# sczhou/CodeFormer

Measured on AMD Instinct MI355X. Metric: aligned 512x512 faces/sec (whole node) at w=0.5, higher is better.
Workload: dtype f32; 1 GPU; BASELINE config 2 (IEEE fp32 arithmetic): 16 faces/GPU, w=0.5, adain, seed-0 random-init weights; global_batch=16, parallelism=single GPU, precision=fp32

## Files before the change

### codeformer_amd/archs/vqgan_arch.py

```python
import torch
import torch.nn.functional as F
from torch import nn

from .. import ops
from ..ops import EPI_RESIDUAL, PRO_AFFINE, PRO_AFFINE_SWISH
from ..utils.logger import get_root_logger
from ..utils.registry import ARCH_REGISTRY
from .hip_module import HipModule

GN_GROUPS = 32
GN_EPS = 1e-6


def normalize(in_channels):
    return nn.GroupNorm(num_groups=GN_GROUPS, num_channels=in_channels, eps=GN_EPS, affine=True)


def swish(x):
    return x * torch.sigmoid(x)


def _gn_tables(norm, *xs, act_growth=None):
    return ops.groupnorm_tables(list(xs), norm.weight, norm.bias, norm.eps, norm.num_groups, act_growth=act_growth)


class VectorQuantizer(HipModule):

    def __init__(self, codebook_size, emb_dim, beta):
        super().__init__()
        self.codebook_size = codebook_size
        self.emb_dim = emb_dim
        self.beta = beta
        self.embedding = nn.Embedding(self.codebook_size, self.emb_dim)
        self.embedding.weight.data.uniform_(-1.0 / self.codebook_size, 1.0 / self.codebook_size)

    def _stats(self, z_q, z, idx, mean_distance):
        enc = torch.zeros(idx.shape[0], self.codebook_size, dtype=z.dtype, device=z.device)
        enc.scatter_(1, idx.view(-1, 1), 1)
        loss = torch.mean((z_q - z) ** 2) * (1.0 + self.beta)
        e_mean = enc.mean(dim=0)
        perplexity = torch.exp(-torch.sum(e_mean * torch.log(e_mean + 1e-10)))
        return loss, {'perplexity': perplexity, 'min_encodings': enc, 'min_encoding_indices': idx.view(-1, 1),
                      'mean_distance': mean_distance}

    def forward(self, z):
        if not z.is_cuda:
            return self.forward_host(z)
        with torch.no_grad():
            B, C, H, W = z.shape
            zt = ops.to_nhwc(z.float()).view(B * H * W, C)
            cb = self.embedding.weight
            pw = self._packed('codebook', lambda: ops.pack_weight(cb), cb)
            idx, _, (scores, zz, ee) = ops.vq_nearest(zt, cb, pw)
            zq_t = ops.codebook_gather(idx, cb, B, H * W)
            z_q = ops.to_nchw(zq_t.view(B, H, W, C))
            loss, stats = self._stats(z_q, z, idx, zz.mean() + ee.mean() - 2.0 * scores.mean())
            return z_q, loss, stats

    def forward_host(self, z):
        zp = z.permute(0, 2, 3, 1).contiguous()
        zf = zp.view(-1, self.emb_dim)
        w = self.embedding.weight
        d = (zf ** 2).sum(dim=1, keepdim=True) + (w ** 2).sum(1) - 2 * torch.matmul(zf, w.t())
        idx = torch.argmin(d, dim=1)
        z_q = w[idx].view(zp.shape)
        z_q = (zp + (z_q - zp).detach()).permute(0, 3, 1, 2).contiguous()
        loss, stats = self._stats(z_q, z, idx, torch.mean(d))
        return z_q, loss, stats

    def get_codebook_feat(self, indices, shape):
        if not indices.is_cuda:
            z_q = self.embedding.weight[indices.view(-1)]
            if shape is not None:
                z_q = z_q.view(shape).permute(0, 3, 1, 2).contiguous()
            return z_q
        with torch.no_grad():
            idx = indices.reshape(-1).contiguous()
            if shape is None:
                return ops.codebook_gather(idx, self.embedding.weight, 1, idx.numel()).view(idx.numel(), -1)
            B, H, W, C = shape
            return ops.to_nchw(ops.codebook_gather(idx, self.embedding.weight, B, H * W).view(B, H, W, C))


class Downsample(HipModule):

    def __init__(self, in_channels):
        super().__init__()
        self.conv = nn.Conv2d(in_channels, in_channels, kernel_size=3, stride=2, padding=0)

    def forward_nhwc(self, x, bf16=False):
        cin, cout = self.conv.in_channels, self.conv.out_channels
        if int(bf16) in (2,) + ops.SPLIT_CODES and ops.split_s2_ok(cin, cout, x.shape[1], x.shape[2]):
            pw = self._packed(('conv', 's2'), lambda: ops.pack_weight(self.conv.weight, self.conv.bias, bf16=ops.SPLIT, stride2=True),
                              self.conv.weight, self.conv.bias)
            return ops.conv2d(x, pw, stride=2, emit_stats=True, act=ops.act_scale(x) if ops.needs_act_scale(pw) else None)
        return ops.conv2d(x, self._pw_conv('conv'), stride=2, emit_stats=True)

    def forward_host(self, x):
        return self.conv(F.pad(x, (0, 1, 0, 1), mode='constant', value=0))


class Upsample(HipModule):

    def __init__(self, in_channels):
        super().__init__()
        self.conv = nn.Conv2d(in_channels, in_channels, kernel_size=3, stride=1, padding=1)

    def forward_nhwc(self, x, bf16=False):
        if int(bf16) == 2:
            bf16 = ops.SPLIT
        c = self.conv.in_channels
        if int(bf16) == ops.WINOGRAD_F43 and x.dtype == torch.float32 and ops.f43_up_ok(c, self.conv.out_channels, 2 * x.shape[1], 2 * x.shape[2]):
            pw = self._packed(('conv', 'f43up'), lambda: ops.pack_weight(self.conv.weight, self.conv.bias, bf16=ops.WF43F), self.conv.weight, self.conv.bias)
            return ops.conv2d(x, pw, upsample=True, emit_stats=True)
        pw = self._pw_conv('conv', bf16, up2x=True, hw=x.shape[1:3])
        return ops.conv2d(x, pw, upsample=True, emit_stats=True, act=ops.act_scale(x) if ops.needs_act_scale(pw) else None)

    def forward_host(self, x):
        return self.conv(F.interpolate(x, scale_factor=2.0, mode='nearest'))


class ResBlock(HipModule):

    def __init__(self, in_channels, out_channels=None):
        super().__init__()
        self.in_channels = in_channels
        self.out_channels = in_channels if out_channels is None else out_channels
        self.norm1 = normalize(in_channels)
        oc = self.out_channels
        self.conv1 = nn.Conv2d(in_channels, oc, kernel_size=3, stride=1, padding=1)
        self.norm2 = normalize(oc)
        self.conv2 = nn.Conv2d(oc, oc, kernel_size=3, stride=1, padding=1)
        if self.in_channels != oc:
            self.conv_out = nn.Conv2d(in_channels, oc, kernel_size=1, stride=1, padding=0)

    def forward_nhwc(self, x, x2=None, bf16=False):
        xs = (x,) if x2 is None else (x, x2)
        sc, sh = _gn_tables(self.norm1, *xs, act_growth=4.0 if self._skip_streams(x, x2, bf16) else None)
        hw = x.shape[1:3]
        npix = hw[0] * hw[1]
        code1 = self._range_code(self.norm1, bf16, npix * self.in_channels // GN_GROUPS)
        code2 = self._range_code(self.norm2, bf16, npix * self.out_channels // GN_GROUPS)
        h = ops.conv2d(x, self._pw_conv('conv1', code1, hw=hw, c_split=None if x2 is None else x.shape[3]), x2=x2, prologue=PRO_AFFINE_SWISH, scale=sc, shift=sh, emit_stats=True)
        sc, sh = _gn_tables(self.norm2, h)
        if self.in_channels != self.out_channels:
            skip = self._skip_nhwc(x, x2, bf16)
        else:
            skip = x
        return ops.conv2d(h, self._pw_conv('conv2', code2, hw=hw), prologue=PRO_AFFINE_SWISH, scale=sc, shift=sh,
                          epilogue=EPI_RESIDUAL, res=skip, emit_stats=True)

    def _skip_streams(self, x, x2, code):
        if self.in_channels == self.out_channels:
            return False
        c_split = None if x2 is None else x.shape[3]
        stored = x.dtype == torch.bfloat16 and getattr(x, '_cf_stats', None) is not None and (x2 is None or getattr(x2, '_cf_stats', None) is not None)
        return bool((int(code) in (2,) + ops.SPLIT_CODES or stored) and ops.RANGE_SCALE and
                    ops.split_1x1_ok(self.in_channels, self.out_channels, x.shape[1], x.shape[2], c_split))

    def _skip_nhwc(self, x, x2, code):
        if self._skip_streams(x, x2, code):
            pw = self._packed(('conv_out', 'f16x2'), lambda: ops.pack_weight(self.conv_out.weight, self.conv_out.bias, bf16=ops.SPLIT),
                              self.conv_out.weight, self.conv_out.bias)
            return ops.conv2d(x, pw, x2=x2, act=ops.act_scale(x, x2))
        return ops.conv2d(x, self._pw_conv('conv_out'), x2=x2)

    def forward_host(self, x_in):
        x = self.conv1(swish(self.norm1(x_in)))
        x = self.conv2(swish(self.norm2(x)))
        if self.in_channels != self.out_channels:
            x_in = self.conv_out(x_in)
        return x + x_in


class AttnBlock(HipModule):

    def __init__(self, in_channels):
        super().__init__()
        self.in_channels = in_channels
        self.norm = normalize(in_channels)
        self.q = nn.Conv2d(in_channels, in_channels, kernel_size=1, stride=1, padding=0)
        self.k = nn.Conv2d(in_channels, in_channels, kernel_size=1, stride=1, padding=0)
        self.v = nn.Conv2d(in_channels, in_channels, kernel_size=1, stride=1, padding=0)
        self.proj_out = nn.Conv2d(in_channels, in_channels, kernel_size=1, stride=1, padding=0)

    def forward_nhwc(self, x):
        B, H, W, C = x.shape
        if H * W != 256:
            raise ValueError(f'AttnBlock HIP path is built for 16x16 feature maps (got {H}x{W})')
        sc, sh = _gn_tables(self.norm, x)
        qkv_w = (self.q.weight, self.k.weight, self.v.weight)
        qkv_b = (self.q.bias, self.k.bias, self.v.bias)
        pw = self._packed('qkv', lambda: ops.pack_weight_cat(qkv_w, qkv_b), *qkv_w, *qkv_b)
        qkv = ops.conv2d(x, pw, prologue=PRO_AFFINE, scale=sc, shift=sh).view(B * 256, 3 * C)
        o = ops.attention(qkv[:, :C], qkv[:, C:2 * C], qkv[:, 2 * C:], B, 1, C, int(C) ** (-0.5))
        return ops.conv2d(o.view(B, H, W, C), self._pw_conv('proj_out'), epilogue=EPI_RESIDUAL, res=x, emit_stats=True)

    def forward_host(self, x):
        h_ = self.norm(x)
        q, k, v = self.q(h_), self.k(h_), self.v(h_)
        b, c, h, w = q.shape
        w_ = torch.bmm(q.reshape(b, c, h * w).permute(0, 2, 1), k.reshape(b, c, h * w)) * (int(c) ** (-0.5))
        w_ = F.softmax(w_, dim=2).permute(0, 2, 1)
        h_ = torch.bmm(v.reshape(b, c, h * w), w_).reshape(b, c, h, w)
        return x + self.proj_out(h_)


class _Conv3x3(HipModule):

    def __init__(self, cin, cout):
        super().__init__()
        conv = nn.Conv2d(cin, cout, kernel_size=3, stride=1, padding=1)
        self.weight, self.bias = conv.weight, conv.bias
        self.in_channels, self.out_channels = cin, cout

    def pw(self, bf16=False):
        return self._packed(('w', int(bf16)), lambda: ops.pack_weight(self.weight, self.bias, bf16=int(bf16)), self.weight,
                            self.bias)

    def forward_nhwc(self, x, bf16=False, **kw):
        plain = not kw.get('out_nchw') and not kw.get('in_nchw')
        if kw.get('img_in') is not None:
            h, w = kw['img_in'].shape[1], kw['img_in'].shape[2]
        else:
            h, w = (x.shape[2], x.shape[3]) if kw.get('in_nchw') else (x.shape[1], x.shape[2])
        unnormalised = plain and kw.get('prologue', ops.PRO_NONE) in (ops.PRO_NONE, ops.PRO_LEAKY)
        if unnormalised and int(bf16) == 2:
            bf16 = ops.SPLIT
        code = ops.conv_code(bf16, self.in_channels, self.out_channels, h, w, plain=plain)
        pw = self.pw(code)
        if unnormalised and ops.needs_act_scale(pw):
            kw['act'] = ops.act_scale(x)
        return ops.conv2d(x, pw, **kw)

    def forward_host(self, x):
        return F.conv2d(x, self.weight, self.bias, stride=1, padding=1)


class _GroupNorm(nn.GroupNorm):

    def forward(self, x):
        if x.is_cuda:
            xn = ops.to_nhwc(x.float())
            sc, sh = ops.groupnorm_tables([xn], self.weight, self.bias, self.eps, self.num_groups)
            B, C = sc.shape
            return x * sc.view(B, C, 1, 1) + sh.view(B, C, 1, 1)
        return super().forward(x)


def _run_blocks_nhwc(blocks, x, taps=None, first_nchw=False, last_nchw=False, bf16=False, storage_bf16=False, img_in=False, img_out=None):
    pending = None
    n = len(blocks)
    for i, blk in enumerate(blocks):
        if storage_bf16 and int(bf16) == 1 and isinstance(blk, Upsample) and x.dtype == torch.float32 and \
                4 * x.shape[1] * x.shape[2] > ops.TOKEN_IMAGE_MAX:
            x = ops.to_bf16(x)
        if isinstance(blk, _GroupNorm):
            pending = ops.groupnorm_tables([x], blk.weight, blk.bias, blk.eps, blk.num_groups) + (blk,)
        elif isinstance(blk, _Conv3x3):
            kw = {}
            code = bf16
            if pending is not None:
                kw.update(prologue=PRO_AFFINE, scale=pending[0], shift=pending[1])
                code = blk._range_code(pending[2], bf16, x.shape[1] * x.shape[2] * x.shape[3] // pending[2].num_groups)
                pending = None
            if i == 0 and first_nchw:
                kw['in_nchw'] = True
                if img_in:
                    x, kw['img_in'] = None, x
            if i == n - 1 and last_nchw:
                kw['out_nchw'] = True
                if img_out is not None:
                    kw['img_out'] = img_out
            kw['emit_stats'] = i != n - 1
            x = blk.forward_nhwc(x, bf16=code, **kw)
        else:
            if pending is not None:
                raise RuntimeError('GroupNorm must be followed by a conv in the block list')
            x = blk.forward_nhwc(x, bf16=bf16) if isinstance(blk, (ResBlock, Upsample, Downsample)) else blk.forward_nhwc(x)
        if taps and i in taps:
            r = taps[i](x)
            if r is not None:
                x = r
    return x


class Encoder(HipModule):

    def __init__(self, in_channels, nf, emb_dim, ch_mult, num_res_blocks, resolution, attn_resolutions):
        super().__init__()
        self.nf = nf
        self.num_resolutions = len(ch_mult)
        self.num_res_blocks = num_res_blocks
        self.resolution = resolution
        self.attn_resolutions = attn_resolutions
        res = resolution
        widths = [nf * m for m in (1,) + tuple(ch_mult)]
        seq = [_Conv3x3(in_channels, nf)]
        ch = nf
        for level in range(self.num_resolutions):
            ch = widths[level]
            for _ in range(num_res_blocks):
                seq.append(ResBlock(ch, widths[level + 1]))
                ch = widths[level + 1]
                if res in attn_resolutions:
                    seq.append(AttnBlock(ch))
            if level != self.num_resolutions - 1:
                seq.append(Downsample(ch))
                res //= 2
        seq += [ResBlock(ch, ch), AttnBlock(ch), ResBlock(ch, ch), _GroupNorm(GN_GROUPS, ch, eps=GN_EPS, affine=True),
                _Conv3x3(ch, emb_dim)]
        self.blocks = nn.ModuleList(seq)

    def forward(self, x):
        if not x.is_cuda:
            return self.forward_host(x)
        with torch.no_grad():
            return ops.to_nchw(self.forward_nhwc(x.float().contiguous()))

    def forward_nhwc(self, x_nchw, taps=None, bf16=False, img_u8=False):
        return _run_blocks_nhwc(self.blocks, x_nchw, taps, first_nchw=True, bf16=bf16, img_in=img_u8)

    def forward_host(self, x):
        for blk in self.blocks:
            x = blk(x)
        return x


class Generator(HipModule):

    def __init__(self, nf, emb_dim, ch_mult, res_blocks, img_size, attn_resolutions):
        super().__init__()
        self.nf = nf
        self.ch_mult = ch_mult
        self.num_resolutions = len(self.ch_mult)
        self.num_res_blocks = res_blocks
        self.resolution = img_size
        self.attn_resolutions = attn_resolutions
        self.in_channels = emb_dim
        self.out_channels = 3
        ch = nf * ch_mult[-1]
        res = img_size // 2 ** (self.num_resolutions - 1)
        seq = [_Conv3x3(emb_dim, ch), ResBlock(ch, ch), AttnBlock(ch), ResBlock(ch, ch)]
        for level in reversed(range(self.num_resolutions)):
            width = nf * ch_mult[level]
            for _ in range(res_blocks):
                seq.append(ResBlock(ch, width))
                ch = width
                if res in attn_resolutions:
                    seq.append(AttnBlock(ch))
            if level != 0:
                seq.append(Upsample(ch))
                res *= 2
        seq += [_GroupNorm(GN_GROUPS, ch, eps=GN_EPS, affine=True), _Conv3x3(ch, self.out_channels)]
        self.blocks = nn.ModuleList(seq)

    def forward(self, x):
        if not x.is_cuda:
            return self.forward_host(x)
        with torch.no_grad():
            return self.forward_nhwc(ops.to_nhwc(x.float()))

    def forward_nhwc(self, x, taps=None, bf16=False, storage_bf16=False, img_out=None):
        return _run_blocks_nhwc(self.blocks, x, taps, last_nchw=True, bf16=bf16, storage_bf16=storage_bf16, img_out=img_out)

    def forward_host(self, x):
        for blk in self.blocks:
            x = blk(x)
        return x


@ARCH_REGISTRY.register()
class VQAutoEncoder(HipModule):

    def __init__(self, img_size, nf, ch_mult, quantizer='nearest', res_blocks=2, attn_resolutions=[16],
                 codebook_size=1024, emb_dim=256, beta=0.25, gumbel_straight_through=False, gumbel_kl_weight=1e-8,
                 model_path=None):
        super().__init__()
        logger = get_root_logger()
        self.in_channels = 3
        self.nf = nf
        self.n_blocks = res_blocks
        self.codebook_size = codebook_size
        self.embed_dim = emb_dim
        self.ch_mult = ch_mult
        self.resolution = img_size
        self.attn_resolutions = attn_resolutions
        self.quantizer_type = quantizer
        self.encoder = Encoder(self.in_channels, nf, emb_dim, ch_mult, res_blocks, img_size, attn_resolutions)
        if quantizer == 'nearest':
            self.beta = beta
            self.quantize = VectorQuantizer(codebook_size, emb_dim, beta)
        else:
            raise NotImplementedError(f"quantizer '{quantizer}' is not part of the MI355X inference path")
        self.generator = Generator(nf, emb_dim, ch_mult, res_blocks, img_size, attn_resolutions)
        if model_path is not None:
            chkpt = torch.load(model_path, map_location='cpu')
            key = 'params_ema' if 'params_ema' in chkpt else ('params' if 'params' in chkpt else None)
            if key is None:
                raise ValueError('Wrong params!')
            self.load_state_dict(chkpt[key])
            logger.info(f'vqgan is loaded from: {model_path} [{key}]')

    def forward(self, x):
        x = self.encoder(x)
        quant, codebook_loss, quant_stats = self.quantize(x)
        x = self.generator(quant)
        return x, codebook_loss, quant_stats
```

### codeformer_amd/csrc/cf_wf43.hip

```cpp
#include <cstdlib>
#include <cstring>
#include <type_traits>

#include "cf_conv_parts.h"




namespace {

constexpr int F4_TH = 16, F4_TW = 16;
constexpr int F4_PW = F4_TW + 2;
constexpr int F4_NPIX = (F4_TH + 2) * F4_PW;
constexpr int F4_SLOTS = F4_NPIX + 4;
constexpr int F4_DUMMY = F4_NPIX;
constexpr int F4_NT = 16;
constexpr int F4_PATCH_FLOATS = F4_SLOTS * CF_BK;
constexpr int F4_PS = F4_NT * CF_BK;
constexpr int F4_V_FLOATS = 36 * F4_PS;
constexpr int F4_M_FLOATS = 36 * 8 * 64;
constexpr int F4_TAB = 256;
constexpr int F4_TAB_32 = 512;
constexpr int F4_LDS_FLOATS = 2 * F4_PATCH_FLOATS + F4_V_FLOATS + 2 * F4_TAB;
static_assert(F4_M_FLOATS <= 2 * F4_PATCH_FLOATS + F4_V_FLOATS, "epilogue staging must fit the patch buffers + V");
static_assert(F4_LDS_FLOATS * 4 <= 81920, "LDS budget of two workgroups per CU");
constexpr int F4_LDS_FLOATS_16 = 2 * F4_M_FLOATS;
static_assert(F4_LDS_FLOATS_16 >= F4_LDS_FLOATS && F4_LDS_FLOATS_16 * 4 <= 163840, "LDS budget of the 16-wave form");
constexpr int F4_LDS_FLOATS_32 = 2 * F4_SLOTS * 32 + 36 * F4_NT * 32 + 2 * F4_TAB_32;
static_assert(F4_LDS_FLOATS_32 >= F4_LDS_FLOATS_16 && F4_LDS_FLOATS_32 * 4 <= 163840, "LDS budget of the 32-channel-slab form");

typedef _Float16 f4_f16x4 __attribute__((ext_vector_type(4)));
typedef float f4_f32x2 __attribute__((ext_vector_type(2)));
typedef unsigned f4_u32x4 __attribute__((ext_vector_type(4)));
typedef unsigned f4_u32x2 __attribute__((ext_vector_type(2)));

__device__ __forceinline__ __amdgpu_buffer_rsrc_t f4_rsrc(const void* p, unsigned bytes) {
  return __builtin_amdgcn_make_buffer_rsrc(const_cast<void*>(p), 0, bytes, 0x00020000);
}
__device__ __forceinline__ f32x4 f4_ld128(__amdgpu_buffer_rsrc_t r, unsigned voff, unsigned soff) {
  return __builtin_bit_cast(f32x4, __builtin_amdgcn_raw_buffer_load_b128(r, (int)voff, (int)soff, 0));
}
__device__ __forceinline__ f4_f32x2 f4_ld64(__amdgpu_buffer_rsrc_t r, unsigned voff, unsigned soff) {
  return __builtin_bit_cast(f4_f32x2, __builtin_amdgcn_raw_buffer_load_b64(r, (int)voff, (int)soff, 0));
}
__device__ __forceinline__ void f4_st64(f4_f32x2 v, __amdgpu_buffer_rsrc_t r, unsigned voff, unsigned soff) {
  __builtin_amdgcn_raw_buffer_store_b64(__builtin_bit_cast(f4_u32x2, v), r, (int)voff, (int)soff, 0);
}

struct F4Args {
  const float* in0;
  const float* in1;
  int c0, c1, cin, nchunks;
  int batch, h, w;
  int cout;
  int prologue, epilogue;
  const float* pro_scale;
  const float* pro_shift;
  const float* weight;
  const float* bias;
  const float* res;
  const float* sft_scale;
  float sft_w;
  float acc_scale;
  const float* act_scale;
  float* out;
  double* stats_out;
  int stats_cpg, nparts;
  int tiles_x, tiles_per_img, ntn;
  int nt_out;
};
static_assert(sizeof(F4Args) == 160, "the kernarg block keeps its size: it feeds the register allocation of every instantiation");

__device__ __forceinline__ int f4_vs(int ty) { return (0x78 >> (2 * ty)) & 3; }

__device__ __forceinline__ unsigned f4_vu(unsigned lq, unsigned p, unsigned t) { return (lq & 1u) + 2u * (((t >> 1) + 4u * (lq >> 1) + p) & 7u); }

template <int PRO, int EPI, int NW, int KS, bool F32, bool UP = false>
__global__ __launch_bounds__(NW * 64, 4) void wf43_kernel(const F4Args a) {
  static_assert(!UP || (F32 && PRO == CF_PRO_NONE && EPI == CF_EPI_NONE), "the upsampling gather: fp32 operands, no prologue, no epilogue operand");
  static_assert(KS == 16 || (KS == 32 && NW == 16), "32-channel slabs need the LDS of the 16-wave form");
  constexpr int F4_THREADS = NW * 64;
  constexpr int F4_BN = NW * 8;
  constexpr int TWV = KS / 4;
  constexpr int QPP = KS / 4;
  constexpr int GT = F4_THREADS - TWV * 64;
  constexpr int F4_APT = 384 * QPP / GT;
  constexpr int PSTEP = GT / QPP;
  constexpr int SLOTB = KS * 4;
  constexpr int PATCHF = F4_SLOTS * KS;
  constexpr int PSK = F4_NT * KS;
  extern __shared__ __attribute__((aligned(16))) float smem[];
  float* const V = smem + 2 * PATCHF;
  constexpr int VBUF = 36 * PSK;
  constexpr int TABN = KS == 32 ? F4_TAB_32 : F4_TAB;
  float* const tab = V + VBUF;

  const int tid = threadIdx.x;
  const int lane = tid & 63;
  const int wave = __builtin_amdgcn_readfirstlane(tid >> 6);

  const int bid = cf_xcd_tile(blockIdx.x, gridDim.x);
  const int ntile = bid % a.ntn;
  const int mt = bid / a.ntn;
  const int n0 = ntile * F4_BN;
  const int b = mt / a.tiles_per_img;
  const int rt = mt - b * a.tiles_per_img;
  const int tyw = rt / a.tiles_x;
  const int y0 = tyw * F4_TH;
  const int x0 = (rt - tyw * a.tiles_x) * F4_TW;
  const int n = a.cin / KS;

  constexpr bool affine = PRO == CF_PRO_AFFINE || PRO == CF_PRO_AFFINE_SWISH;
  if (affine) {
    for (int i = tid; i < a.cin; i += F4_THREADS) {
      tab[i] = a.pro_scale[(size_t)b * a.cin + i];
      tab[TABN + i] = a.pro_shift[(size_t)b * a.cin + i];
    }
  }
  float act_s, act_is, act_s02;
  cf_act_scales<!affine>(a.act_scale, b, act_s, act_is, act_s02);

  const int pix_origin = (y0 - 1) * a.w + (x0 - 1);
  auto item = [&](unsigned u, int j, unsigned& rel, bool& valid) __attribute__((always_inline)) {
    const unsigned p = u + (unsigned)(PSTEP * j);
    const unsigned hy = (p * 3641u) >> 16;
    const unsigned hx = p - 18u * hy;
    const int iy = y0 - 1 + (int)hy, ix = x0 - 1 + (int)hx;
    valid = (int)(p < (unsigned)F4_NPIX) & (int)((unsigned)iy < (unsigned)a.h) & (int)((unsigned)ix < (unsigned)a.w);
    if constexpr (UP) {
      const unsigned sy = valid ? (unsigned)iy : (unsigned)(y0 + 8), sx = valid ? (unsigned)ix : (unsigned)(x0 + 8);
      rel = (sy >> 1) * ((unsigned)a.w >> 1) + (sx >> 1);
    } else {
      rel = valid ? hy * (unsigned)a.w + hx : (unsigned)(9 * a.w + 9);
    }
  };
  const size_t img0 = (size_t)b * a.h * a.w;
  const unsigned img_px = (unsigned)(a.h * a.w);
  const size_t img0_in = UP ? img0 / 4 : img0;
  const unsigned img_px_in = UP ? img_px / 4 : img_px;
  const __amdgpu_buffer_rsrc_t rs_in0 = f4_rsrc(a.in0 + img0_in * a.c0, img_px_in * (unsigned)a.c0 * 4u);
  const __amdgpu_buffer_rsrc_t rs_in1 = f4_rsrc(a.c1 ? a.in1 + img0_in * a.c1 : a.in0, img_px_in * (unsigned)a.c1 * 4u);
  constexpr bool HALVES = F4_APT >= 6;
  constexpr int RAN = HALVES ? F4_APT / 2 : F4_APT;
  f32x4 ra[RAN], rb[HALVES ? RAN : 1];
  auto load_A_range = [&](int chunk, auto j0c, auto j1c) __attribute__((always_inline)) {
    constexpr int J0 = decltype(j0c)::value, J1 = decltype(j1c)::value;
    const int c = chunk * KS;
    const bool first = c < a.c0;
    const unsigned cs = (unsigned)(first ? a.c0 : a.c1);
    const unsigned soff = (unsigned)(first ? c : c - a.c0) * 4u;
    unsigned tl = (unsigned)tid - (unsigned)(TWV * 64);
    asm volatile("" : "+v"(tl));
    const unsigned k4x = (tl % (unsigned)QPP) * 4u;
#pragma unroll
    for (int j = J0; j < J1; ++j) {
      unsigned rel;
      bool valid;
      item(tl / (unsigned)QPP, j, rel, valid);
      const unsigned voff = (__umul24(UP ? rel : (unsigned)(pix_origin + (int)rel), cs) + k4x) * 4u;
      (HALVES && j >= RAN ? rb[j % RAN] : ra[j % RAN]) = first ? f4_ld128(rs_in0, voff, soff) : f4_ld128(rs_in1, voff, soff);
    }
  };
  auto load_A = [&](int chunk) __attribute__((always_inline)) { load_A_range(chunk, std::integral_constant<int, 0>{}, std::integral_constant<int, F4_APT>{}); };
  auto store_patch_range = [&](int chunk, auto j0c, auto j1c) __attribute__((always_inline)) {
    constexpr int J0 = decltype(j0c)::value, J1 = decltype(j1c)::value;
    unsigned tl = (unsigned)tid - (unsigned)(TWV * 64);
    asm volatile("" : "+v"(tl));
    const unsigned k4 = tl % (unsigned)QPP, slot = tl / (unsigned)QPP;
    char* const pb = reinterpret_cast<char*>(smem + (chunk & 1) * PATCHF) + (((slot & ~3u) | ((slot ^ (slot >> 2)) & 3u)) * (unsigned)SLOTB + k4 * 16u);
    f32x4 sc = {1.f, 1.f, 1.f, 1.f}, sh = {0.f, 0.f, 0.f, 0.f};
    if (affine) {
      sc = *reinterpret_cast<const f32x4*>(tab + chunk * KS + k4 * 4);
      sh = *reinterpret_cast<const f32x4*>(tab + TABN + chunk * KS + k4 * 4);
    }
#pragma unroll
    for (int j = J0; j < J1; ++j) {
      unsigned rel;
      bool valid;
      item(slot, j, rel, valid);
      const f32x4 v = cf_pro_apply4<PRO, true>(HALVES && j >= RAN ? rb[j % RAN] : ra[j % RAN], sc, sh, act_s, act_s02, valid);
      if (j < F4_APT - 1 || slot + (unsigned)(PSTEP * j) < (unsigned)F4_NPIX) *reinterpret_cast<f32x4*>(pb + j * (PSTEP * SLOTB)) = v;
    }
  };

  auto store_patch = [&](int chunk) __attribute__((always_inline)) { store_patch_range(chunk, std::integral_constant<int, 0>{}, std::integral_constant<int, F4_APT>{}); };

  const int tg = (wave >> (KS == 32 ? 2 : 1)) & 1;
  float* t_hi;
  float* t_lo;
  auto row_pass = [&](const f4_f32x2 (&zz)[6], int pos) __attribute__((always_inline)) {
    f4_f32x2 v[6];
    v[0] = (zz[0] + zz[4]) * 0.25f - zz[2] * 1.0625f;
    const f4_f32x2 e1 = zz[4] * 0.25f - zz[2];
    const f4_f32x2 o1 = zz[3] * 0.125f - zz[1] * 0.5f;
    v[1] = e1 + o1;
    v[2] = e1 - o1;
    const f4_f32x2 e2 = zz[4] * 0.5f - zz[2] * 0.125f;
    const f4_f32x2 o2 = zz[3] - zz[1] * 0.25f;
    v[3] = e2 + o2;
    v[4] = e2 - o2;
    v[5] = (zz[1] + zz[5]) * 0.25f - zz[3] * 1.0625f;
#pragma unroll
    for (int nu = 0; nu < 6; ++nu) {
      if (F32) {
        t_hi[(pos + nu) * PSK] = v[nu][0];
        t_lo[(pos + nu) * PSK] = v[nu][1];
      } else {
        float hi, lo;
        cf_split_pair(v[nu][0], v[nu][1], hi, lo);
        t_hi[(pos + nu) * PSK] = hi;
        t_lo[(pos + nu) * PSK] = lo;
      }
    }
  };
  auto transform = [&](int chunk, auto mid) __attribute__((always_inline)) {
    const char* const pb = reinterpret_cast<const char*>(smem + (chunk & 1) * PATCHF);
    unsigned ln = (unsigned)lane;
    asm volatile("" : "+v"(ln));
    const unsigned t_tile = KS == 32 ? 4u * (unsigned)(wave & 3) + (ln >> 4) : 8u * (unsigned)(wave & 1) + (ln >> 3);
    const unsigned t_cp = KS == 32 ? ln & 15u : ln & 7u;
    const unsigned t_ty = t_tile >> 2, t_tx = t_tile & 3u;
    constexpr unsigned SH = KS == 32 ? 7 : 6;
    const unsigned t_base = (4u << SH) * (18u * t_ty + t_tx) + t_cp * 8u;
    const unsigned tb0 = 2u * t_ty + t_tx;
    unsigned tk[4];
#pragma unroll
    for (int k = 0; k < 4; ++k) tk[k] = t_base | (((tb0 + k) & 3u) << SH);
    if (F32) {
      const unsigned lq0 = (2u * t_cp) & 3u, j = t_cp >> 1;
      if (KS == 32) {
        t_hi = V + (tg * 18) * PSK + t_tile * 32 + f4_vu(lq0, j >> 1, t_tile) * 2u + (j & 1u);
        t_lo = V + (tg * 18) * PSK + t_tile * 32 + f4_vu(lq0 + 1u, j >> 1, t_tile) * 2u + (j & 1u);
      } else {
        t_hi = V + (tg * 18) * PSK + t_tile * CF_BK + ((lq0 ^ (unsigned)f4_vs((int)t_ty)) << 2) + j;
        t_lo = V + (tg * 18) * PSK + t_tile * CF_BK + (((lq0 + 1u) ^ (unsigned)f4_vs((int)t_ty)) << 2) + j;
      }
    } else if (KS == 32) {
      const unsigned lq = t_cp >> 2, e = t_cp & 3u;
      t_hi = V + (tg * 18) * PSK + t_tile * 32 + f4_vu(lq, e >> 1, t_tile) * 2u + (e & 1u);
      t_lo = V + (tg * 18) * PSK + t_tile * 32 + f4_vu(lq, 2u + (e >> 1), t_tile) * 2u + (e & 1u);
    } else {
      t_hi = V + (tg * 18) * PSK + t_tile * CF_BK + (((t_cp >> 1) ^ (unsigned)f4_vs((int)t_ty)) << 2) + (t_cp & 1u);
      t_lo = t_hi + 2;
    }
    auto px = [&](int r, int j) __attribute__((always_inline)) {
      const int q = 2 * r + j;
      return *reinterpret_cast<const f4_f32x2*>(pb + (4 << SH) * (4 * r + (q >> 2)) + (tk[q >> 2] ^ (((unsigned)q & 3u) << SH)));
    };
    if (tg == 0) {
      {
        f4_f32x2 z[6];
#pragma unroll
        for (int j = 0; j < 6; ++j) z[j] = (px(0, j) + px(4, j)) * 0.25f - px(2, j) * 1.0625f;
        __builtin_amdgcn_sched_barrier(0);
        row_pass(z, 0);
      }
      __builtin_amdgcn_sched_barrier(0);
      {
        f4_f32x2 zp[6], zm[6];
#pragma unroll
        for (int j = 0; j < 6; ++j) {
          const f4_f32x2 e = px(4, j) * 0.25f - px(2, j);
          const f4_f32x2 o = px(3, j) * 0.125f - px(1, j) * 0.5f;
          zp[j] = e + o;
          zm[j] = e - o;
          if (j == 2) __builtin_amdgcn_sched_barrier(0);
        }
        __builtin_amdgcn_sched_barrier(0);
        row_pass(zp, 6);
        __builtin_amdgcn_sched_barrier(0);
        mid();
        __builtin_amdgcn_sched_barrier(0);
        row_pass(zm, 12);
      }
    } else {
      {
        f4_f32x2 z[6];
#pragma unroll
        for (int j = 0; j < 6; ++j) z[j] = (px(1, j) + px(5, j)) * 0.25f - px(3, j) * 1.0625f;
        __builtin_amdgcn_sched_barrier(0);
        row_pass(z, 12);
      }
      __builtin_amdgcn_sched_barrier(0);
      {
        f4_f32x2 zp[6], zm[6];
#pragma unroll
        for (int j = 0; j < 6; ++j) {
          const f4_f32x2 e = px(4, j) * 0.5f - px(2, j) * 0.125f;
          const f4_f32x2 o = px(3, j) - px(1, j) * 0.25f;
          zp[j] = e + o;
          zm[j] = e - o;
          if (j == 2) __builtin_amdgcn_sched_barrier(0);
        }
        __builtin_amdgcn_sched_barrier(0);
        row_pass(zp, 0);
        __builtin_amdgcn_sched_barrier(0);
        mid();
        __builtin_amdgcn_sched_barrier(0);
        row_pass(zm, 6);
      }
    }
  };

  const int m_g = wave / (NW / 2), m_nb = wave % (NW / 2);
  f32x4 acc[18];
#pragma unroll
  for (int i = 0; i < 18; ++i) acc[i] = f32x4{0.f, 0.f, 0.f, 0.f};
  const __amdgpu_buffer_rsrc_t rs_w = f4_rsrc(a.weight, 36u * (unsigned)a.cin * (unsigned)a.cout * 4u);
  const unsigned w_pos = (unsigned)a.cin * (unsigned)a.cout * 4u;
  const unsigned w_chunk = (unsigned)(a.cout * KS) * 4u;
  const unsigned w_s0 = (unsigned)(18 * m_g) * w_pos + (unsigned)(n0 / 16 + m_nb) * (unsigned)(64 * KS);
  constexpr std::integral_constant<int, 4> nb4{};
  unsigned lane16;
  f32x4 bq[4];
  auto load_B = [&](int chunk, int i, auto nb) __attribute__((always_inline)) {
    bq[i % decltype(nb)::value] = f4_ld128(rs_w, lane16, w_s0 + (unsigned)i * w_pos + (unsigned)chunk * w_chunk);
  };
  auto set_lane16 = [&]() __attribute__((always_inline)) {
    unsigned ln = (unsigned)lane;
    asm volatile("" : "+v"(ln));
    lane16 = ln * 16u;
  };
  const float* a_base;
  f32x4 va[4];
  auto mfma = [&](float a0, float a1, float b0, float b1, f32x4& c) __attribute__((always_inline)) {
    c = __builtin_amdgcn_mfma_f32_16x16x16f16(__builtin_bit_cast(f4_f16x4, f4_f32x2{a0, a1}), __builtin_bit_cast(f4_f16x4, f4_f32x2{b0, b1}), c, 0, 0, 0);
  };
  auto mma_stage = [&](int chunk, auto na, auto after_last_B) __attribute__((always_inline)) {
    constexpr int NA = decltype(na)::value;
    {
      unsigned ln = (unsigned)lane;
      asm volatile("" : "+v"(ln));
      const unsigned t15 = ln & 15u;
      a_base = V + (18 * m_g) * PSK + t15 * CF_BK + (((ln >> 4) ^ (unsigned)f4_vs((int)(t15 >> 2))) << 2);
      lane16 = ln * 16u;
    }
    auto read_A = [&](int i) __attribute__((always_inline)) { va[i % NA] = *reinterpret_cast<const f32x4*>(a_base + i * PSK); };
    read_A(0);
    read_A(1);
#pragma unroll
    for (int i = 0; i < 18; i += 2) {
      if (NA == 4 && i + 2 < 18) {
        read_A(i + 2);
        read_A(i + 3);
      }
      __builtin_amdgcn_sched_barrier(0);
      const f32x4 a0 = va[i % NA], a1 = va[(i + 1) % NA], b0 = bq[i % 4], b1 = bq[(i + 1) % 4];
      if (F32) {
#pragma unroll
        for (int j = 0; j < 4; ++j) {
          acc[i] = __builtin_amdgcn_mfma_f32_16x16x4f32(a0[j], b0[j], acc[i], 0, 0, 0);
          acc[i + 1] = __builtin_amdgcn_mfma_f32_16x16x4f32(a1[j], b1[j], acc[i + 1], 0, 0, 0);
        }
      } else {
        mfma(a0[2], a0[3], b0[0], b0[1], acc[i]);
        mfma(a1[2], a1[3], b1[0], b1[1], acc[i + 1]);
        mfma(a0[0], a0[1], b0[2], b0[3], acc[i]);
        mfma(a1[0], a1[1], b1[2], b1[3], acc[i + 1]);
        mfma(a0[0], a0[1], b0[0], b0[1], acc[i]);
        mfma(a1[0], a1[1], b1[0], b1[1], acc[i + 1]);
      }
      if (NA == 2 && i + 2 < 18) {
        read_A(i + 2);
        read_A(i + 3);
      }
      if (i + 4 < 18) {
        load_B(chunk, i + 4, nb4);
        load_B(chunk, i + 5, nb4);
      }
      if (i + 4 == 16) after_last_B();
      __builtin_amdgcn_sched_barrier(0);
    }
  };
  typedef _Float16 f4_f16x8 __attribute__((ext_vector_type(8)));
  f32x4 xb[3][2], xa[1][2];
  const int p_g = 18 * m_g;
  const int p_nb = m_nb;
  const unsigned w_s32 = (unsigned)p_g * w_pos + (unsigned)(n0 / 16 + p_nb) * (unsigned)(64 * KS);
  auto load_B32 = [&](int chunk, int i) __attribute__((always_inline)) {
    const unsigned so = w_s32 + (unsigned)i * w_pos + (unsigned)chunk * w_chunk;
    xb[i % 3][0] = f4_ld128(rs_w, lane16, so);
    xb[i % 3][1] = f4_ld128(rs_w, lane16 + 16u, so);
  };
  auto mma_stage32 = [&](int chunk) __attribute__((always_inline)) {
    unsigned ao[4];
    {
      unsigned ln = (unsigned)lane;
      asm volatile("" : "+v"(ln));
      const unsigned t15 = ln & 15u, lq = ln >> 4;
#pragma unroll
      for (unsigned pp = 0; pp < 4; ++pp) ao[pp] = ((unsigned)p_g * (unsigned)PSK + t15 * 32u + f4_vu(lq, pp, t15) * 2u) * 4u;
      lane16 = ln * 32u;
    }
    const char* const vb = reinterpret_cast<const char*>(V);
    auto read_A = [&](int pos) __attribute__((always_inline)) {
      const f4_f32x2 p0 = *reinterpret_cast<const f4_f32x2*>(vb + ao[0] + pos * (PSK * 4)), p1 = *reinterpret_cast<const f4_f32x2*>(vb + ao[1] + pos * (PSK * 4));
      const f4_f32x2 p2 = *reinterpret_cast<const f4_f32x2*>(vb + ao[2] + pos * (PSK * 4)), p3 = *reinterpret_cast<const f4_f32x2*>(vb + ao[3] + pos * (PSK * 4));
      xa[0][0] = f32x4{p0[0], p0[1], p1[0], p1[1]};
      xa[0][1] = f32x4{p2[0], p2[1], p3[0], p3[1]};
    };
    auto mf = [&](f32x4 av, f32x4 bv, f32x4& c) __attribute__((always_inline)) {
      c = __builtin_amdgcn_mfma_f32_16x16x32_f16(__builtin_bit_cast(f4_f16x8, av), __builtin_bit_cast(f4_f16x8, bv), c, 0, 0, 0);
    };
    read_A(0);
#pragma unroll
    for (int i = 0; i < 18; ++i) {
      __builtin_amdgcn_sched_barrier(0);
      if (F32) {
#pragma unroll
        for (int j = 0; j < 8; ++j) {
          acc[i] = __builtin_amdgcn_mfma_f32_16x16x4f32(xa[0][j >> 2][j & 3], xb[i % 3][j >> 2][j & 3], acc[i], 0, 0, 0);
        }
      } else {
        mf(xa[0][1], xb[i % 3][0], acc[i]);
        mf(xa[0][0], xb[i % 3][1], acc[i]);
        mf(xa[0][0], xb[i % 3][0], acc[i]);
      }
      if (i + 1 < 18) read_A(i + 1);
      if (i + 3 < 18) load_B32(chunk, i + 3);
      __builtin_amdgcn_sched_barrier(0);
    }
  };
  auto set_lane32 = [&]() __attribute__((always_inline)) {
    unsigned ln = (unsigned)lane;
    asm volatile("" : "+v"(ln));
    lane16 = ln * 32u;
  };
  constexpr std::integral_constant<int, 4> na4{};
  constexpr std::integral_constant<int, 4> na_gather{};
  auto feed = [&](int s) __attribute__((always_inline)) {
    if (s < n) {
      store_patch(s);
    }
  };

  if constexpr (KS == 32) {
    if (wave < TWV) {
      __syncthreads();
      __syncthreads();
      for (int s = 0; s < n; ++s) {
        transform(s, [&]() __attribute__((always_inline)) {
          set_lane32();
          load_B32(s, 0);
        });
        __builtin_amdgcn_sched_barrier(0);
        load_B32(s, 1);
        load_B32(s, 2);
        __builtin_amdgcn_sched_barrier(0);
        __syncthreads();
        mma_stage32(s);
        __builtin_amdgcn_sched_barrier(0);
        __syncthreads();
      }
    } else {
      constexpr std::integral_constant<int, 0> h0{};
      constexpr std::integral_constant<int, F4_APT / 2> h1{};
      constexpr std::integral_constant<int, F4_APT> h2{};
      auto feed2 = [&](int s) __attribute__((always_inline)) {
        if (s < n) {
          load_A_range(s, h1, h2);
          __builtin_amdgcn_sched_barrier(0);
          store_patch_range(s, h0, h1);
          __builtin_amdgcn_sched_barrier(0);
          store_patch_range(s, h1, h2);
        }
      };
      load_A_range(0, h0, h1);
      __syncthreads();
      feed2(0);
      if (n > 1) load_A_range(1, h0, h1);
      __syncthreads();
      for (int s = 0; s < n; ++s) {
        feed2(s + 1);
        __builtin_amdgcn_sched_barrier(0);
        set_lane32();
#pragma unroll
        for (int i = 0; i < 3; ++i) load_B32(s, i);
        __builtin_amdgcn_sched_barrier(0);
        __syncthreads();
        mma_stage32(s);
        __builtin_amdgcn_sched_barrier(0);
        if (s + 2 < n) load_A_range(s + 2, h0, h1);
        __builtin_amdgcn_sched_barrier(0);
        __syncthreads();
      }
    }
  } else if (wave < 4) {
    __syncthreads();
    __syncthreads();
    for (int s = 0; s < n; ++s) {
      transform(s, [&]() __attribute__((always_inline)) {
        set_lane16();
        load_B(s, 0, nb4);
        load_B(s, 1, nb4);
      });
      __builtin_amdgcn_sched_barrier(0);
      load_B(s, 2, nb4);
      load_B(s, 3, nb4);
      __builtin_amdgcn_sched_barrier(0);
      __syncthreads();
      mma_stage(s, na4, []() __attribute__((always_inline)) {});
      __builtin_amdgcn_sched_barrier(0);
      __syncthreads();
    }
  } else {
    constexpr std::integral_constant<int, 0> h0{};
    constexpr std::integral_constant<int, (HALVES ? F4_APT / 2 : F4_APT)> h1{};
    constexpr std::integral_constant<int, F4_APT> h2{};
    auto feedh = [&](int s) __attribute__((always_inline)) {
      if (s < n) {
        if (HALVES) load_A_range(s, h1, h2);
        __builtin_amdgcn_sched_barrier(0);
        store_patch_range(s, h0, h1);
        __builtin_amdgcn_sched_barrier(0);
        if (HALVES) store_patch_range(s, h1, h2);
      }
    };
    load_A_range(0, h0, h1);
    __syncthreads();
    feedh(0);
    if (n > 1) load_A_range(1, h0, h1);
    __syncthreads();
    int s = 0;
    for (; s + 2 < n; ++s) {
      feedh(s + 1);
      __builtin_amdgcn_sched_barrier(0);
      set_lane16();
#pragma unroll
      for (int i = 0; i < 4; ++i) load_B(s, i, nb4);
      __builtin_amdgcn_sched_barrier(0);
      __syncthreads();
      mma_stage(s, na_gather, [&]() __attribute__((always_inline)) { load_A_range(s + 2, h0, h1); });
      __builtin_amdgcn_sched_barrier(0);
      __syncthreads();
    }
    for (; s < n; ++s) {
      feedh(s + 1);
      __builtin_amdgcn_sched_barrier(0);
      set_lane16();
#pragma unroll
      for (int i = 0; i < 4; ++i) load_B(s, i, nb4);
      __builtin_amdgcn_sched_barrier(0);
      __syncthreads();
      mma_stage(s, na_gather, []() __attribute__((always_inline)) {});
      __builtin_amdgcn_sched_barrier(0);
      __syncthreads();
    }
  }

  float* const Mst = smem;
  const int e_cp = (lane & 31) + 32 * (wave >> 3), e_rh = lane >> 5, e_tp = wave & 7;
  const float acc_s = a.acc_scale * act_is;
  const int nn = n0 + 2 * e_cp;
  f4_f32x2 bias2 = {0.f, 0.f};
  if (a.bias) bias2 = *reinterpret_cast<const f4_f32x2*>(a.bias + nn);
  const unsigned e_rowc = (unsigned)a.w * (unsigned)a.cout * 4u;
  const unsigned e_px = (unsigned)a.cout * 4u;
  const unsigned e_img = img_px * (unsigned)a.cout * 4u;
  const __amdgpu_buffer_rsrc_t rs_out = f4_rsrc(a.out + img0 * a.cout, e_img);
  const __amdgpu_buffer_rsrc_t rs_res = f4_rsrc(EPI == CF_EPI_NONE ? a.out : a.res + img0 * a.cout, e_img);
  const __amdgpu_buffer_rsrc_t rs_sft = f4_rsrc(EPI == CF_EPI_SFT ? a.sft_scale + img0 * a.cout : a.out, e_img);
  const bool rh1 = e_rh != 0;
  const float ca1 = rh1 ? 0.25f : 1.f, ca2 = rh1 ? 4.f : 1.f, cb1 = rh1 ? 0.125f : 0.5f, cb2 = rh1 ? 8.f : 2.f;
  double psum = 0.0, psq = 0.0;
#pragma unroll
  for (int th = 0; th < 2; ++th) {
    unsigned e_zero = 0;
    asm volatile("" : "+v"(e_zero));
    const unsigned voff0 = (unsigned)(2 * e_rh) * e_rowc + (unsigned)(2 * e_cp) * 4u + e_zero;
    const unsigned soff0 = (unsigned)(y0 + 4 * (e_tp >> 1)) * e_rowc + (unsigned)(x0 + 4 * (2 * th + (e_tp & 1))) * e_px + (unsigned)n0 * 4u;
    f4_f32x2 r0[2][4], r1[2][4];
#pragma unroll
    for (int aa = 0; aa < 2; ++aa)
#pragma unroll
      for (int c = 0; c < 4; ++c) {
        r0[aa][c] = r1[aa][c] = f4_f32x2{0.f, 0.f};
        if (EPI == CF_EPI_RESIDUAL || EPI == CF_EPI_SFT) r0[aa][c] = f4_ld64(rs_res, voff0, soff0 + aa * e_rowc + c * e_px);
      }
    __builtin_amdgcn_sched_barrier(0);
    if (th > 0) __syncthreads();
#pragma unroll
    for (int i = 0; i < 18; ++i) {
      float* mp = Mst + ((18 * m_g + i) * 8 + 2 * (lane >> 4)) * F4_BN + m_nb * 16 + (lane & 15);
      mp[0] = acc[i][2 * th];
      mp[F4_BN] = acc[i][2 * th + 1];
    }
    if (EPI == CF_EPI_SFT) {
#pragma unroll
      for (int aa = 0; aa < 2; ++aa)
#pragma unroll
        for (int c = 0; c < 4; ++c) r1[aa][c] = f4_ld64(rs_sft, voff0, soff0 + aa * e_rowc + c * e_px);
    }
    __syncthreads();
    const float* mq = Mst + e_tp * F4_BN + 2 * e_cp;
    auto col = [&](int nu, f4_f32x2& tA, f4_f32x2& tB) __attribute__((always_inline)) {
      auto m = [&](int xi) __attribute__((always_inline)) { return *reinterpret_cast<const f4_f32x2*>(mq + ((xi * 6 + nu) * 8) * F4_BN); };
      const f4_f32x2 m1 = m(1), m2 = m(2), m3 = m(3), m4 = m(4);
      const f4_f32x2 me = *reinterpret_cast<const f4_f32x2*>(mq + (((rh1 ? 5 : 0) * 6 + nu) * 8) * F4_BN);
      const f4_f32x2 s1 = m1 + m2, d1 = m1 - m2, s2 = m3 + m4, d2 = m3 - m4;
      const f4_f32x2 x = s1 * ca1 + s2 * ca2, y = d1 * cb1 + d2 * cb2;
      const f4_f32x2 xm = x + me, ym = y + me;
      tA = rh1 ? x : xm;
      tB = rh1 ? ym : y;
    };
    f4_f32x2 o[2][4];
    {
      f4_f32x2 t0[2], ta[2], tb[2];
      col(0, t0[0], t0[1]);
      col(1, ta[0], ta[1]);
      col(2, tb[0], tb[1]);
#pragma unroll
      for (int aa = 0; aa < 2; ++aa) {
        const f4_f32x2 s = ta[aa] + tb[aa], d = ta[aa] - tb[aa];
        o[aa][0] = t0[aa] + s;
        o[aa][1] = d * 0.5f;
        o[aa][2] = s * 0.25f;
        o[aa][3] = d * 0.125f;
      }
      col(3, ta[0], ta[1]);
      col(4, tb[0], tb[1]);
      col(5, t0[0], t0[1]);
#pragma unroll
      for (int aa = 0; aa < 2; ++aa) {
        const f4_f32x2 s = ta[aa] + tb[aa], d = ta[aa] - tb[aa];
        o[aa][0] += s;
        o[aa][1] += d * 2.f;
        o[aa][2] += s * 4.f;
        o[aa][3] += d * 8.f + t0[aa];
      }
    }
    double dsum = 0.0, dsq = 0.0, dsum1 = 0.0, dsq1 = 0.0;
#pragma unroll
    for (int aa = 0; aa < 2; ++aa) {
      f4_f32x2 rs = {0.f, 0.f}, rq = {0.f, 0.f};
#pragma unroll
      for (int c = 0; c < 4; ++c) {
        f4_f32x2 v = o[aa][c] * acc_s + bias2;
        if (EPI == CF_EPI_RESIDUAL) v += r0[aa][c];
        else if (EPI == CF_EPI_SFT) v = r0[aa][c] + a.sft_w * (r0[aa][c] * r1[aa][c] + v);
        o[aa][c] = v;
        rs += v;
        rq += v * v;
      }
      dsum += (double)rs[0];
      dsq += (double)rq[0];
      dsum1 += (double)rs[1];
      dsq1 += (double)rq[1];
    }
    if (a.nt_out) {
#pragma unroll
      for (int aa = 0; aa < 2; ++aa)
#pragma unroll
        for (int c = 0; c < 4; ++c)
          __builtin_amdgcn_raw_buffer_store_b64(__builtin_bit_cast(f4_u32x2, o[aa][c]), rs_out, (int)voff0, (int)(soff0 + aa * e_rowc + c * e_px), 2);
    } else {
#pragma unroll
      for (int aa = 0; aa < 2; ++aa)
#pragma unroll
        for (int c = 0; c < 4; ++c) f4_st64(o[aa][c], rs_out, voff0, soff0 + aa * e_rowc + c * e_px);
    }
    if (a.stats_out) {
      const int cpg = a.stats_cpg;
      dsum += dsum1;
      dsq += dsq1;
      dsum += __shfl_xor(dsum, 32, 64);
      dsq += __shfl_xor(dsq, 32, 64);
      for (int o2 = 1; o2 * 2 < cpg; o2 <<= 1) {
        dsum += __shfl_xor(dsum, o2, 64);
        dsq += __shfl_xor(dsq, o2, 64);
      }
      psum = th == 0 ? dsum : psum + dsum;
      psq = th == 0 ? dsq : psq + dsq;
    }
  }
  if (a.stats_out) {
    const int cpg = a.stats_cpg;
    double* const sred = reinterpret_cast<double*>(smem);
    __syncthreads();
    if (e_rh == 0) {
      sred[(wave * 32 + (lane & 31)) * 2] = psum;
      sred[(wave * 32 + (lane & 31)) * 2 + 1] = psq;
    }
    __syncthreads();
    if (e_tp == 0 && e_rh == 0 && (nn % cpg) == 0) {
      double s0 = 0.0, s1 = 0.0;
#pragma unroll
      for (int wv = 0; wv < 8; ++wv) {
        s0 += sred[((wave + wv) * 32 + (lane & 31)) * 2];
        s1 += sred[((wave + wv) * 32 + (lane & 31)) * 2 + 1];
      }
      double* op = cf_gn_partial_ptr(a.stats_out, b, a.cout, cpg, nn, a.nparts, rt);
      op[0] = s0;
      op[1] = s1;
    }
  }
}

__global__ void pack_weight_wf43_kernel(const float* __restrict__ w, int cout, int cin, int cout_pad, int nchunks, float scale,
                                        unsigned* __restrict__ packed, long total, int k32, int f32) {
  const long i = (long)blockIdx.x * blockDim.x + threadIdx.x;
  if (i >= total) return;
  if (f32) {
    const int j = k32 ? (int)(i & 7) : (int)(i & 3), ln = k32 ? (int)((i >> 3) & 63) : (int)((i >> 2) & 63);
    long r = k32 ? i >> 9 : i >> 8;
    const int ntiles = cout_pad / 16;
    const int nn = (int)(r % ntiles) * 16 + (ln & 15);
    r /= ntiles;
    const int chunk = (int)(r % nchunks), pos = (int)(r / nchunks);
    const int c = chunk * (k32 ? 32 : CF_BK) + 4 * j + (ln >> 4);
    const int xi = pos / 6, nu = pos % 6;
    const double Gf[6][3] = {{4.0, 0.0, 0.0},           {-32.0 / 15.0, -16.0 / 15.0, -8.0 / 15.0}, {-32.0 / 15.0, 16.0 / 15.0, -8.0 / 15.0},
                             {1.0 / 15.0, 2.0 / 15.0, 4.0 / 15.0}, {1.0 / 15.0, -2.0 / 15.0, 4.0 / 15.0},  {0.0, 0.0, 4.0}};
    float val = 0.f;
    if (nn < cout && c < cin) {
      const float* g = w + ((long)nn * cin + c) * 9;
      double u = 0.0;
#pragma unroll
      for (int y = 0; y < 3; ++y) {
        double rowv = 0.0;
#pragma unroll
        for (int x = 0; x < 3; ++x) rowv += (double)g[y * 3 + x] * Gf[nu][x];
        u += Gf[xi][y] * rowv;
      }
      val = (float)u;
    }
    packed[i] = __builtin_bit_cast(unsigned, val);
    return;
  }
  const int e = k32 ? (int)(i & 3) : (int)(i & 1), part = k32 ? (int)((i >> 2) & 1) : (int)((i >> 1) & 1);
  const int ln = k32 ? (int)((i >> 3) & 63) : (int)((i >> 2) & 63);
  long r = k32 ? i >> 9 : i >> 8;
  const int ntiles = cout_pad / 16;
  const int nn = (int)(r % ntiles) * 16 + (ln & 15);
  r /= ntiles;
  const int chunk = (int)(r % nchunks);
  const int pos = (int)(r / nchunks);
  const int xi = pos / 6, nu = pos % 6;
  const double Gm[6][3] = {{4.0, 0.0, 0.0},           {-32.0 / 15.0, -16.0 / 15.0, -8.0 / 15.0}, {-32.0 / 15.0, 16.0 / 15.0, -8.0 / 15.0},
                           {1.0 / 15.0, 2.0 / 15.0, 4.0 / 15.0}, {1.0 / 15.0, -2.0 / 15.0, 4.0 / 15.0},  {0.0, 0.0, 4.0}};
  unsigned out = 0;
#pragma unroll
  for (int h = 0; h < 2; ++h) {
    const int c = k32 ? chunk * 32 + (ln >> 4) * 8 + e * 2 + h : chunk * CF_BK + (ln >> 4) * 4 + e * 2 + h;
    float val = 0.f;
    if (nn < cout && c < cin) {
      const float* g = w + ((long)nn * cin + c) * 9;
      double u = 0.0;
#pragma unroll
      for (int y = 0; y < 3; ++y) {
        double rowv = 0.0;
#pragma unroll
        for (int x = 0; x < 3; ++x) rowv += (double)g[y * 3 + x] * Gm[nu][x];
        u += Gm[xi][y] * rowv;
      }
      val = (float)(u * (double)scale);
    }
    const _Float16 hi = (_Float16)val;
    const _Float16 hv = part ? (_Float16)(val - (float)hi) : hi;
    out |= (unsigned)__builtin_bit_cast(unsigned short, hv) << (16 * h);
  }
  packed[i] = out;
}

}

static int f4_wide_mode() {
  static const int v = [] {
    const char* w = getenv("CF_F43_WIDE");
    if (!w || !strcmp(w, "k32")) return 1;
    if (!strcmp(w, "k16")) return 0;
    fprintf(stderr, "libcodeformer_hip: CF_F43_WIDE=%s is not a form of the 16-wave F(4,3) workgroup (k32 | k16): using k32\n", w);
    return 1;
  }();
  return v;
}
static bool f4_k32_enabled() { return f4_wide_mode() == 1; }

extern "C" int cf_pack_conv_weight_winograd43_f16x2(const float* w, int cout, int cin, int cout_pad, int cin_pad, float scale, void* packed,
                                                    cf_stream_t stream) {
  CF_REQUIRE(w && packed, "cf_pack_conv_weight_winograd43_f16x2: null pointer");
  CF_REQUIRE(cin_pad % CF_BK == 0 && cin_pad >= cin && cout_pad >= cout && cout_pad % 64 == 0,
             "cf_pack_conv_weight_winograd43_f16x2: bad padding cin %d->%d cout %d->%d", cin, cin_pad, cout, cout_pad);
  int ex = 0;
  CF_REQUIRE(scale > 0.f && frexpf(scale, &ex) == 0.5f, "cf_pack_conv_weight_winograd43_f16x2: scale %g is not a power of two", (double)scale);
  const long total = 36L * cin_pad * cout_pad;
  const int k32 = cout_pad % 128 == 0 && cin_pad % 32 == 0 && f4_k32_enabled();
  hipLaunchKernelGGL(pack_weight_wf43_kernel, dim3((unsigned)((total + 255) / 256)), dim3(256), 0, (hipStream_t)stream, w, cout, cin,
                     cout_pad, cin_pad / (k32 ? 32 : CF_BK), scale, reinterpret_cast<unsigned*>(packed), total, k32, 0);
  CF_CHECK_LAUNCH("cf_pack_conv_weight_winograd43_f16x2");
  return CF_OK;
}

extern "C" int cf_pack_conv_weight_winograd43(const float* w, int cout, int cin, int cout_pad, int cin_pad, void* packed, cf_stream_t stream) {
  CF_REQUIRE(w && packed, "cf_pack_conv_weight_winograd43: null pointer");
  CF_REQUIRE(cin_pad % CF_BK == 0 && cin_pad >= cin && cout_pad >= cout && cout_pad % 64 == 0,
             "cf_pack_conv_weight_winograd43: bad padding cin %d->%d cout %d->%d", cin, cin_pad, cout, cout_pad);
  const long total = 36L * cin_pad * cout_pad;
  const int k32 = cout_pad % 128 == 0 && cin_pad % 32 == 0 && f4_k32_enabled();
  hipLaunchKernelGGL(pack_weight_wf43_kernel, dim3((unsigned)((total + 255) / 256)), dim3(256), 0, (hipStream_t)stream, w, cout, cin,
                     cout_pad, cin_pad / (k32 ? 32 : CF_BK), 1.f, reinterpret_cast<unsigned*>(packed), total, k32, 1);
  CF_CHECK_LAUNCH("cf_pack_conv_weight_winograd43");
  return CF_OK;
}

int cf_wf43_launch(const cf_conv_desc* d, hipStream_t stream, int* parts_query) {
  CF_REQUIRE(d->taps == 9 && d->stride == 1 && !d->in_nchw && !d->out_nchw &&
                 (d->bf16_mfma == CF_OPERAND_F16X2 || d->bf16_mfma == CF_OPERAND_F32),
             "cf_conv2d(winograd 2): F(4x4,3x3) covers 3x3 stride-1 NHWC convolutions with split-half or fp32 operands");
  const bool f32 = d->bf16_mfma == CF_OPERAND_F32;
  CF_REQUIRE(!d->upsample || (f32 && d->prologue == CF_PRO_NONE && d->epilogue == CF_EPI_NONE && d->c1 == 0 && d->cout % 128 == 0 && d->c0 % 32 == 0 &&
                              f4_k32_enabled()),
             "cf_conv2d(winograd 2, upsample): fp32 operands, one input with c0 %% 32 == 0, cout %% 128 == 0, no prologue / epilogue operand");
  if (!f32)
    if (const int e = cf_require_acc_scale(d, "cf_conv2d(winograd 2)")) return e;
  CF_REQUIRE(!f32 || !d->act_scale, "cf_conv2d(winograd 2): fp32 operands take no activation range scale");
  CF_REQUIRE(d->hout % F4_TH == 0 && d->wout % F4_TW == 0, "cf_conv2d(winograd 2): needs an output of %dx%d multiples (got %dx%d)", F4_TH,
             F4_TW, d->hout, d->wout);
  CF_REQUIRE(d->cout % 64 == 0 && d->cout_pad == d->cout, "cf_conv2d(winograd 2): needs cout == cout_pad, a multiple of 64 (got %d / %d)",
             d->cout, d->cout_pad);
  CF_REQUIRE((long)d->hout * d->wout <= (1L << 21), "cf_conv2d(winograd 2): at most 2^21 pixels per image (got %dx%d)", d->hout, d->wout);
  CF_REQUIRE((long)d->hout * d->wout * (d->c0 > d->cout ? d->c0 : d->cout) * 4 < (1L << 31) && (long)d->hout * d->wout * d->c1 * 4 < (1L << 31),
             "cf_conv2d(winograd 2): an image of a tensor must stay below 2^31 bytes (%dx%d, %d / %d / %d channels)", d->hout, d->wout, d->c0, d->c1, d->cout);
  const int tab_max = (d->cout % 128 == 0 && (d->c0 + d->c1) % 32 == 0 && f4_k32_enabled()) ? F4_TAB_32 : F4_TAB;
  CF_REQUIRE(d->c0 + d->c1 <= tab_max, "cf_conv2d(winograd 2): at most %d input channels in this form (got %d)", tab_max, d->c0 + d->c1);
  CF_REQUIRE(cf_epi_is_quad_triple(d), "cf_conv2d(winograd 2): epilogues are none / residual / SFT");
  CF_REQUIRE(cf_dense_zero_pad(d) && d->split_k < 1, "cf_conv2d(winograd 2): reads / writes dense tensors with zero padding, no split_k");
  CF_REQUIRE(d->stats_cpg == 0 || (d->stats_cpg <= 64 && (d->stats_cpg & (d->stats_cpg - 1)) == 0 && d->stats_cpg >= 2),
             "cf_conv2d(winograd 2): stats_cpg %d (a power of two, 2..64)", d->stats_cpg);
  F4Args a;
  cf_fill_conv_args(a, d);
  a.nchunks = a.cin / CF_BK;
  a.h = d->hout;
  a.w = d->wout;
  a.acc_scale = f32 ? 1.f : d->acc_scale;
  a.act_scale = d->act_scale;
  a.stats_cpg = d->stats_cpg > 0 ? d->stats_cpg : 2;
  a.tiles_x = d->wout / F4_TW;
  a.tiles_per_img = a.tiles_x * (d->hout / F4_TH);
  a.nparts = a.tiles_per_img;
  const bool wide = d->cout % 128 == 0;
  const bool k32 = wide && (d->c0 + d->c1) % 32 == 0 && f4_k32_enabled();
  CF_REQUIRE(!k32 || d->c0 % 32 == 0, "cf_conv2d(winograd 2): with cout %% 128 == 0 and cin %% 32 == 0 the concat boundary must be a multiple of 32 (c0 = %d)", d->c0);
  a.ntn = d->cout / (wide ? 128 : 64);
  a.nt_out = cf_nt_store((long)d->batch * d->hout * d->wout * d->cout * 4);
  if (parts_query) {
    *parts_query = a.nparts;
    return CF_OK;
  }
  const size_t lds = (k32 ? F4_LDS_FLOATS_32 : wide ? F4_LDS_FLOATS_16 : F4_LDS_FLOATS) * sizeof(float);
  const dim3 grid(a.tiles_per_img * d->batch * a.ntn), block(wide ? 1024 : 512);
  if (d->upsample) {
    CF_LDS_ATTR((wf43_kernel<CF_PRO_NONE, CF_EPI_NONE, 16, 32, true, true>), F4_LDS_FLOATS_32 * sizeof(float));
    hipLaunchKernelGGL((wf43_kernel<CF_PRO_NONE, CF_EPI_NONE, 16, 32, true, true>), grid, block, lds, stream, a);
    CF_CHECK_LAUNCH("cf_conv2d(winograd F(4,3) fp32, upsampling gather)");
    return CF_OK;
  }
  auto launch = [&](auto pro, auto epi, auto op) {
    constexpr int P = decltype(pro)::value, E = decltype(epi)::value;
    constexpr bool O = decltype(op)::value;
    CF_LDS_ATTR((wf43_kernel<P, E, 8, 16, O>), F4_LDS_FLOATS * sizeof(float));
    CF_LDS_ATTR((wf43_kernel<P, E, 16, 16, O>), F4_LDS_FLOATS_16 * sizeof(float));
    CF_LDS_ATTR((wf43_kernel<P, E, 16, 32, O>), F4_LDS_FLOATS_32 * sizeof(float));
    if (k32) hipLaunchKernelGGL((wf43_kernel<P, E, 16, 32, O>), grid, block, lds, stream, a);
    else if (wide) hipLaunchKernelGGL((wf43_kernel<P, E, 16, 16, O>), grid, block, lds, stream, a);
    else hipLaunchKernelGGL((wf43_kernel<P, E, 8, 16, O>), grid, block, lds, stream, a);
  };
  cf_with_prologue(d->prologue, [&](auto pro) {
    cf_with_epilogue(d->epilogue, [&](auto epi) {
      if (f32) launch(pro, epi, std::true_type{});
      else launch(pro, epi, std::false_type{});
    });
  });
  CF_CHECK_LAUNCH("cf_conv2d(winograd F(4,3) f16x2)");
  return CF_OK;
}
```

### codeformer_amd/lib.py

```python
import ctypes
import os

import torch

_PKG = os.path.dirname(os.path.abspath(__file__))
LIB_PATH = os.environ.get('CF_LIB_PATH') or os.path.join(_PKG, 'libcodeformer_hip.so')

c_float_p = ctypes.c_void_p

ABI_VERSION = 22
PRO_NONE, PRO_AFFINE, PRO_AFFINE_SWISH, PRO_LEAKY = 0, 1, 2, 3
EPI_NONE, EPI_RESIDUAL, EPI_SFT, EPI_GELU, EPI_LEAKY, EPI_AXPY, EPI_AXPY2 = 0, 1, 2, 3, 4, 5, 6
PAD_ZERO, PAD_REFLECT, PAD_EDGE = 0, 1, 2


class ConvDesc(ctypes.Structure):
    _fields_ = [
        ('in0', ctypes.c_void_p), ('in1', ctypes.c_void_p),
        ('c0', ctypes.c_int32), ('c1', ctypes.c_int32),
        ('batch', ctypes.c_int32), ('hin', ctypes.c_int32), ('win', ctypes.c_int32),
        ('hout', ctypes.c_int32), ('wout', ctypes.c_int32),
        ('cout', ctypes.c_int32), ('cout_pad', ctypes.c_int32),
        ('taps', ctypes.c_int32), ('stride', ctypes.c_int32), ('upsample', ctypes.c_int32),
        ('in_nchw', ctypes.c_int32), ('out_nchw', ctypes.c_int32),
        ('prologue', ctypes.c_int32), ('epilogue', ctypes.c_int32),
        ('pro_scale', ctypes.c_void_p), ('pro_shift', ctypes.c_void_p),
        ('weight', ctypes.c_void_p), ('bias', ctypes.c_void_p),
        ('res', ctypes.c_void_p), ('sft_scale', ctypes.c_void_p),
        ('sft_w', ctypes.c_float),
        ('out', ctypes.c_void_p),
        ('stats_out', ctypes.c_void_p), ('stats_cpg', ctypes.c_int32), ('bf16_mfma', ctypes.c_int32),
        ('ld_in0', ctypes.c_int32), ('ld_in1', ctypes.c_int32), ('ld_out', ctypes.c_int32),
        ('pad_mode', ctypes.c_int32), ('pad_lo', ctypes.c_int32), ('winograd', ctypes.c_int32),
        ('acc_scale', ctypes.c_float),
        ('split_k', ctypes.c_int32), ('workspace', ctypes.c_void_p), ('counters', ctypes.c_void_p),
        ('act_scale', ctypes.c_void_p),
        ('io_bf16', ctypes.c_int32),
        ('in0_alt', ctypes.c_void_p), ('alt_cout0', ctypes.c_int32),
    ]


_I, _P, _F, _L = ctypes.c_int, ctypes.c_void_p, ctypes.c_float, ctypes.c_int64
SIGNATURES = {
    'cf_version': (_I, []),
    'cf_last_error': (ctypes.c_char_p, []),
    'cf_build_id': (ctypes.c_char_p, []),
    'cf_device_cu_count': (_I, []),
    'cf_device_init': (_I, []),
    'cf_conv2d': (_I, [ctypes.POINTER(ConvDesc), _P]),
    'cf_conv2d_u8': (_I, [ctypes.POINTER(ConvDesc), _P, _P, _P]),
    'cf_conv2d_stats_parts': (_I, [ctypes.POINTER(ConvDesc)]),
    'cf_conv2d_workspace_bytes': (_L, [ctypes.POINTER(ConvDesc)]),
    'cf_conv2d_tiles': (_I, [ctypes.POINTER(ConvDesc)]),
    'cf_pack_conv_weight': (_I, [_P, _I, _I, _I, _I, _I, _P, _P]),
    'cf_packed_weight_elems': (_L, [_I, _I, _I]),
    'cf_pack_conv_weight_bf16': (_I, [_P, _I, _I, _I, _I, _I, _P, _P]),
    'cf_pack_conv_weight_f16': (_I, [_P, _I, _I, _I, _I, _I, _P, _P]),
    'cf_pack_conv_weight_up2x': (_I, [_P, _I, _I, _I, _I, _P, _P]),
    'cf_pack_conv_weight_winograd': (_I, [_P, _I, _I, _I, _I, _P, _P]),
    'cf_pack_conv_weight_winograd_f16x2': (_I, [_P, _I, _I, _I, _I, _F, _P, _P]),
    'cf_pack_conv_weight_winograd_bf16': (_I, [_P, _I, _I, _I, _I, _F, _P, _P]),
    'cf_pack_conv_weight_winograd43_f16x2': (_I, [_P, _I, _I, _I, _I, _F, _P, _P]),
    'cf_pack_conv_weight_winograd43': (_I, [_P, _I, _I, _I, _I, _P, _P]),
    'cf_pack_linear_weight_f16x2': (_I, [_P, _I, _I, _F, _P, _P]),
    'cf_pack_conv_weight_up2x_bf16': (_I, [_P, _I, _I, _I, _I, _P, _P]),
    'cf_pack_conv_weight_up2x_f16': (_I, [_P, _I, _I, _I, _I, _P, _P]),
    'cf_pack_conv_weight_f16x2': (_I, [_P, _I, _I, _I, _I, _I, _F, _P, _P]),
    'cf_groupnorm_stats': (_I, [_P, _I, _I, _I, _I, _P, _I, _P]),
    'cf_act_scale_from_stats': (_I, [_P, _I, _I, _F, _P, _P, _P]),
    'cf_act_scale_from_tensor': (_I, [_P, _I, _L, _F, _P, _P, _P]),
    'cf_act_scale_fused': (_I, [_P, _I, _P, _I, _P, _L, _I, _F, _P, _P, _P]),
    'cf_groupnorm_finalize': (_I, [_P, _I, _I, _I, _I, _I, _L, _P, _P, _F, _P, _P, _I, _P]),
    'cf_groupnorm_finalize2': (_I, [_P, _I, _I, _I, _I, _P, _I, _I, _I, _I, _I, _L, _P, _P, _F, _P, _P, _I, _F, _P, _P, _P]),
    'cf_layernorm': (_I, [_P, _I, _I, _P, _P, _F, _P, _I, _P, _P, _P]),
    'cf_attention': (_I, [_P, _I, _P, _I, _P, _I, _P, _I, _I, _I, _I, _I, _F, _P]),
    'cf_argmax_rows': (_I, [_P, _I, _I, _P, _P]),
    'cf_argmax_rows_gap': (_I, [_P, _I, _I, _I, _P, _P, _P, _P]),
    'cf_codebook_gather_adain': (_I, [_P, _P, _I, _P, _I, _I, _I, _I, _F, _P, _P]),
    'cf_row_sqnorm': (_I, [_P, _I, _I, _P, _P]),
    'cf_vq_argmin': (_I, [_P, _P, _P, _I, _I, _P, _P, _P]),
    'cf_nchw_to_nhwc': (_I, [_P, _I, _I, _I, _P, _P]),
    'cf_pixel_unshuffle_nhwc': (_I, [_P, _I, _I, _I, _I, _I, _I, _P, _P]),
    'cf_nhwc_to_nchw': (_I, [_P, _I, _I, _I, _P, _P]),
    'cf_img_u8_to_tensor': (_I, [_P, _I, _I, _I, _P, _P]),
    'cf_tensor_to_img_u8': (_I, [_P, _I, _I, _I, _P, _P]),
    'cf_mask_composite': (_I, [_P, _P, _I, _I, _I, _P, _P]),
    'cf_f32_to_bf16': (_I, [_P, _L, _P, _P]),
    'cf_fused_bias_act': (_I, [_P, _P, _L, _I, _I, _F, _F, _P, _P]),
    'cf_fused_bias_act_ex': (_I, [_P, _P, _P, _L, _I, _I, _I, _I, _F, _F, _I, _P, _P]),
    'cf_upfirdn2d': (_I, [_P, _I, _I, _I, _P, _I, _I, _I, _I, _I, _I, _I, _I, _I, _I, _P, _P]),
    'cf_warp_affine_u8': (_I, [_P, _L, _I, _I, _P, _I, _P, _I, _I, _I, _I, _I, _I, _I, _I, _I, _P]),
    'cf_warp_affine_f32': (_I, [_P, _I, _I, ctypes.POINTER(ctypes.c_double), _P, _I, _I, _I, _I, _P]),
    'cf_erode_f32': (_I, [_P, _P, _P, _I, _I, _I, _P]),
    'cf_gaussian_blur_f32': (_I, [_P, _P, _P, _I, _I, _I, _I, _I, _I, _P, _I, _P]),
    'cf_sum_f32': (_I, [_P, _L, _P, _P]),
    'cf_paste_blend': (_I, [_P, _I, _I, _P, _I, _I, ctypes.POINTER(ctypes.c_double), _P, _P, _P, _I, _I, _I, _I, _P]),
    'cf_resize_linear_u8': (_I, [_P, _I, _I, _P, _I, _I, _P]),
    'cf_resize_area_u8': (_I, [_P, _I, _I, _P, _I, _I, _P]),
    'cf_f32_to_u8_trunc': (_I, [_P, _L, _P, _P]),
    'cf_label_lut_f32': (_I, [_P, _L, ctypes.POINTER(ctypes.c_float), _I, _P, _P]),
    'cf_scale_clear_border_f32': (_I, [_P, _I, _I, _I, _I, _F, _P]),
    'cf_box_overlay_u8': (_I, [_P, _I, _I, _P, _I, _I, _I, _P, _P]),
    'cf_resize_linear_f32': (_I, [_P, _I, _I, _I, _P, _I, _I, _P]),
    'cf_esrgan_tile_gather_u8': (_I, [_P, _I, _I, _I, _I, _I, _I, _I, _I, _I, _P, _P]),
    'cf_esrgan_tile_scatter_u8': (_I, [_P, _I, _I, _I, _I, _I, _I, _I, _P, _I, _I, _I, _I, _P]),
}

_lib = None
_cuda = None
_devices = set()


class NativeLibraryError(RuntimeError):
    pass


def load():
    global _cuda
    lib = _lib if _lib is not None else _open()
    if _cuda is None:
        _cuda = torch.cuda.is_available()
    if _cuda:
        dev = torch.cuda.current_device()
        if dev not in _devices:
            _init_device(lib, dev)
    return lib


def _init_device(lib, dev):
    if torch.cuda.is_current_stream_capturing():
        raise NativeLibraryError(f'cf_device_init has not run on cuda:{dev} yet and the current stream is capturing: call '
                                 'codeformer_amd.lib.ensure_device(device) (or run one forward) before the capture')
    if lib.cf_device_init() != 0:
        raise NativeLibraryError(f'cf_device_init failed on cuda:{dev} ({torch.cuda.get_device_name(dev)}): '
                                 f'{lib.cf_last_error().decode("utf-8", "replace")}')
    _devices.add(dev)


def ensure_device(device):
    global _cuda
    lib = _lib if _lib is not None else _open()
    if _cuda is None:
        _cuda = torch.cuda.is_available()
    if not _cuda:
        return lib
    d = torch.device(device) if not isinstance(device, int) else torch.device('cuda', device)
    idx = torch.cuda.current_device() if d.index is None else d.index
    if idx not in _devices:
        with torch.cuda.device(idx):
            _init_device(lib, idx)
    return lib


def _open():
    global _lib
    if not os.path.exists(LIB_PATH):
        raise NativeLibraryError(
            f'{LIB_PATH} not found: build it with `python -m codeformer_amd.build` (hipcc --offload-arch=gfx950). '
            'codeformer_amd has no non-HIP execution path for GPU tensors.')
    try:
        lib = ctypes.CDLL(LIB_PATH)
    except OSError as e:
        raise NativeLibraryError(f'cannot load {LIB_PATH}: {e}') from e
    for name, (res, args) in SIGNATURES.items():
        fn = getattr(lib, name)
        fn.restype = res
        fn.argtypes = args
    if lib.cf_version() != ABI_VERSION:
        raise NativeLibraryError(f'ABI version mismatch: library {lib.cf_version()}, binding {ABI_VERSION}')
    _lib = lib
    return lib


def is_available():
    return os.path.exists(LIB_PATH)


def last_error():
    lib = _lib if _lib is not None else _open()
    return lib.cf_last_error().decode('utf-8', 'replace')


def check(status, what):
    if status != 0:
        raise RuntimeError(f'{what} failed ({status}): {last_error()}')


def stream_ptr():
    return torch.cuda.current_stream().cuda_stream


def ptr(t, strided=False, dtype=torch.float32):
    if t is None:
        return None
    if not t.is_cuda:
        raise ValueError('codeformer_amd ops need CUDA (ROCm) tensors')
    if dtype is not None and t.dtype != dtype:
        raise TypeError(f'codeformer_amd op expected a {dtype} tensor, got {t.dtype}')
    if not strided and not t.is_contiguous():
        raise ValueError('codeformer_amd ops need contiguous tensors')
    return t.data_ptr()
```

### codeformer_amd/ops.py

```python
import ctypes
import math
import os
import weakref

import torch

from . import lib as L
from .lib import (EPI_AXPY, EPI_AXPY2, EPI_GELU, EPI_LEAKY, EPI_NONE, EPI_RESIDUAL, EPI_SFT, PRO_AFFINE, PRO_AFFINE_SWISH,
                  PAD_EDGE, PAD_REFLECT, PAD_ZERO, PRO_LEAKY, PRO_NONE)

GN_GROUPS = 32
GN_EPS = 1e-6

PROFILE = None


def _f32(t):
    if t.dtype != torch.float32:
        raise TypeError(f'expected float32, got {t.dtype}')
    return t


def _act_dtype(t, what='activation'):
    if t.dtype not in (torch.float32, torch.bfloat16):
        raise TypeError(f'{what}: expected float32 or bfloat16, got {t.dtype}')
    return t.dtype


def to_bf16(x):
    if x.dtype == torch.bfloat16:
        return x
    _f32(x)
    if not x.is_contiguous() or x.numel() % 8:
        raise ValueError('to_bf16: expected a dense tensor with a multiple of 8 elements')
    y = torch.empty(x.shape, dtype=torch.bfloat16, device=x.device)
    L.check(L.load().cf_f32_to_bf16(L.ptr(x), x.numel(), L.ptr(y, dtype=torch.bfloat16), L.stream_ptr()), 'cf_f32_to_bf16')
    for attr in ('_cf_stats', '_cf_act'):
        v = getattr(x, attr, None)
        if v is not None:
            setattr(y, attr, v)
    return y


class GNStats:

    __slots__ = ('part', 'parts', 'cpg')

    def __init__(self, part, parts, cpg):
        self.part, self.parts, self.cpg = part, parts, cpg


class PackedWeight:

    __slots__ = ('w', 'bias', 'cout', 'cin', 'taps', 'cout_pad', 'cin_pad', 'bf16', 'up2x', 'wino', 'scale', 's2', 'conv1')

    def __init__(self, w, bias, cout, cin, taps, cout_pad, cin_pad, bf16=False, up2x=False, wino=False, scale=1.0, s2=False, conv1=False):
        self.w, self.bias, self.cout, self.cin, self.taps = w, bias, cout, cin, taps
        self.cout_pad, self.cin_pad, self.bf16, self.up2x, self.wino = cout_pad, cin_pad, bf16, up2x, wino
        self.s2 = s2
        self.conv1 = conv1
        self.scale = scale


def _cout_pad(cout):
    if cout <= 32:
        return 32
    if cout <= 64:
        return 64
    return (cout + 127) // 128 * 128


WINOGRAD = 3
SPLIT = 4
WSPLIT = 6
GSPLIT = 7
WF16 = 8
WBF16 = 9
SPLIT_F43 = 10
WF43 = 11
WINOGRAD_F43 = 12
WF43F = 13
OPERAND_F16X2 = 3
SPLIT_CODES = (SPLIT, SPLIT_F43)


def split_ok(cin, cout, hin, win, c_split=None):
    return cin % 32 == 0 and cout % 64 == 0 and hin % 16 == 0 and win % 16 == 0 and (c_split is None or c_split % 32 == 0)


def split_s2_ok(cin, cout, hin, win):
    return cin % 16 == 0 and cout % 64 == 0 and hin % 16 == 0 and win % 32 == 0


def split_1x1_ok(cin, cout, h, w, c_split=None):
    return cin % 32 == 0 and cout % 64 == 0 and h % 8 == 0 and w % 16 == 0 and h * w > TOKEN_IMAGE_MAX and (c_split is None or c_split % 32 == 0)


def winograd_ok(cin, cout, hout, wout):
    return cin % 16 == 0 and cout % 64 == 0 and hout % 8 == 0 and wout % 16 == 0


F43_WIDE_MIN_PIXELS = 128 * 128
F43_WIDE_MIN_PIXELS_FP32 = 64 * 64


def f43_ok(cin, cout, hout, wout, fp32=False):
    if cout != 64 and (cout % 128 or hout * wout < (F43_WIDE_MIN_PIXELS_FP32 if fp32 else F43_WIDE_MIN_PIXELS)):
        return False
    cin_max = 512 if (cout % 128 == 0 and cin % 32 == 0) else 256
    return cin % 16 == 0 and cin <= cin_max and cout % 64 == 0 and hout % 16 == 0 and wout % 16 == 0




def f43_up_ok(cin, cout, hout, wout):
    return cin % 32 == 0 and cin <= 256 and cout % 128 == 0 and hout % 16 == 0 and wout % 16 == 0 and \
        hout * wout >= F43_WIDE_MIN_PIXELS_FP32


SPLIT_MIN_PIXELS = 32 * 32
TOKEN_IMAGE_MAX = 1024


def wsingle_ok(cin, cout, h, w):
    return winograd_ok(cin, cout, h, w) and cout % 128 == 0 and h * w >= SPLIT_MIN_PIXELS


def c_split_ok(c_split, slab):
    return c_split is None or c_split % slab == 0


def conv_code(code, cin, cout, h, w, up2x=False, c_split=None, plain=True):
    code = int(code)
    f43_slab = 32 if (cout % 128 == 0 and cin % 32 == 0) else 16
    if code == WINOGRAD_F43:
        if plain and not up2x and c_split_ok(c_split, f43_slab) and f43_ok(cin, cout, h, w, fp32=True):
            return WF43F
        code = WINOGRAD
    if code == SPLIT_F43:
        if plain and not up2x and c_split_ok(c_split, f43_slab) and f43_ok(cin, cout, h, w):
            return WF43
        code = SPLIT
    if code == SPLIT:
        if plain and not up2x and winograd_ok(cin, cout, h, w):
            return WSPLIT
        if plain and split_ok(cin, cout, h, w, c_split) and (up2x or h * w >= SPLIT_MIN_PIXELS):
            return SPLIT
        code = WINOGRAD
    if code == WINOGRAD:
        return WINOGRAD if (plain and not up2x and winograd_ok(cin, cout, h, w)) else 0
    if code and not (plain and cin % 32 == 0 and cout % 4 == 0):
        return 0
    if code in (1, 2) and plain and not up2x and wsingle_ok(cin, cout, h, w):
        return WBF16 if code == 1 else WF16
    return code


RANGE_SCALE = os.environ.get('CODEFORMER_HIP_RANGE_SCALE', '1') != '0'
HALF_LIMIT = 65504.0 / 4.0


def switches():
    return (RANGE_SCALE, FINALIZE_FUSED)


def needs_act_scale(pw):
    if pw.conv1:
        return RANGE_SCALE
    return RANGE_SCALE and pw.taps == 9 and int(pw.bf16) in (1, 2, OPERAND_F16X2) and (bool(pw.wino) or int(pw.bf16) == OPERAND_F16X2)


_ACT_CELLS = {}


def _act_cells(device, batch):
    key = (str(device), torch.cuda.current_stream(device).cuda_stream)
    t = _ACT_CELLS.get(key)
    if t is None or t.numel() < 2 * batch:
        t = torch.zeros(max(2 * batch, 256), dtype=torch.int32, device=device)
        _ACT_CELLS[key] = t
    return t


def tensor_version(t):
    return None if t.is_inference() else t._version


def act_scale(x, x2=None, growth=4.0):
    ver = tensor_version(x)
    if ver is None and getattr(x, '_cf_stats', None) is not None:
        ver = 'inference'
    if x2 is None and ver is not None:
        cached = getattr(x, '_cf_act', None)
        if cached is not None and cached[0] == (float(growth), ver):
            return cached[1]
    if x2 is not None:
        cached = getattr(x, '_cf_act_pair', None)
        if cached is not None and cached[2]() is x2 and cached[0] == _act_key(x, growth) and cached[1] == _act_key(x2, growth):
            return cached[3]
    lib = L.load()
    B = x.shape[0]
    act = torch.empty(B, 2, dtype=torch.float32, device=x.device)
    cells = L.ptr(_act_cells(x.device, B), dtype=torch.int32)
    st = getattr(x, '_cf_stats', None)
    st2 = None if x2 is None else getattr(x2, '_cf_stats', None)
    if x2 is not None and (st is None or st2 is None):
        a1, a2 = act_scale(x, growth=growth), act_scale(x2, growth=growth)
        return torch.stack((torch.minimum(a1[:, 0], a2[:, 0]), torch.maximum(a1[:, 1], a2[:, 1])), dim=1)
    if st is not None:
        nper = st.part.numel() // (2 * B)
        p2, n2 = (L.ptr(st2.part, dtype=torch.float64), st2.part.numel() // (2 * B)) if st2 is not None else (None, 0)
        L.check(lib.cf_act_scale_fused(L.ptr(st.part, dtype=torch.float64), nper, p2, n2, None, 0, B, float(growth), cells, L.ptr(act), L.stream_ptr()),
                'cf_act_scale_fused')
    else:
        if not x.is_contiguous() or (x.numel() // B) % 4:
            raise ValueError('act_scale: expected a dense tensor with a multiple of 4 elements per image')
        L.check(lib.cf_act_scale_fused(None, 0, None, 0, L.ptr(_f32(x)), x.numel() // B, B, float(growth), cells, L.ptr(act), L.stream_ptr()),
                'cf_act_scale_fused')
    if x2 is None and ver is not None:
        x._cf_act = ((float(growth), ver), act)
    return act


class StatsPair:

    def __init__(self):
        self.buf, self.n, self.used = None, 0, 0

    def take(self, n, device):
        if self.buf is None:
            self.buf, self.n = torch.empty(2 * n, dtype=torch.float64, device=device), n
        if n != self.n or self.used >= 2:
            raise ValueError('StatsPair: two launches of equal statistics size')
        self.used += 1
        return self.buf[(self.used - 1) * n:self.used * n]


def act_scale_pair(pair, batch, growth=4.0):
    if pair.used != 2:
        raise ValueError('act_scale_pair: the pair has not been filled by two launches')
    lib = L.load()
    act = torch.empty(2 * batch, 2, dtype=torch.float32, device=pair.buf.device)
    cells = L.ptr(_act_cells(pair.buf.device, 2 * batch), dtype=torch.int32)
    L.check(lib.cf_act_scale_fused(L.ptr(pair.buf, dtype=torch.float64), pair.n // (2 * batch), None, 0, None, 0, 2 * batch, float(growth), cells, L.ptr(act),
                                   L.stream_ptr()), 'cf_act_scale_fused')
    return act[:batch], act[batch:]


def gn_range_ok(gmax, bmax, n):
    return gmax * math.sqrt(max(n - 1, 1)) + bmax < HALF_LIMIT


def exact_code(code):
    code = int(code)
    return {SPLIT: WINOGRAD, SPLIT_F43: WINOGRAD, 2: WINOGRAD}.get(code, code)


def pack_scale(wmax):
    return 1.0 if wmax == 0.0 or not math.isfinite(wmax) else 2.0 ** (14 - math.frexp(wmax)[1] + 1)


def _f23_max(w):
    g = w.double()
    r = torch.stack((g[:, :, 0], 0.5 * (g[:, :, 0] + g[:, :, 1] + g[:, :, 2]), 0.5 * (g[:, :, 0] - g[:, :, 1] + g[:, :, 2]), g[:, :, 2]), dim=2)
    u = torch.stack((r[..., 0], 0.5 * (r[..., 0] + r[..., 1] + r[..., 2]), 0.5 * (r[..., 0] - r[..., 1] + r[..., 2]), r[..., 2]), dim=3)
    return float(u.abs().max())


def _f43_max(w):
    Gm = torch.tensor([[4.0, 0.0, 0.0], [-32 / 15, -16 / 15, -8 / 15], [-32 / 15, 16 / 15, -8 / 15], [1 / 15, 2 / 15, 4 / 15],
                       [1 / 15, -2 / 15, 4 / 15], [0.0, 0.0, 4.0]], dtype=torch.float64, device=w.device)
    return float(torch.einsum('xa,kcab,yb->kcxy', Gm, w.double(), Gm).abs().max())


def _require_3x3(w, cin_mult, cout_mult, what, up2x):
    if up2x or w.dim() != 4 or tuple(w.shape[2:]) != (3, 3) or w.shape[1] % cin_mult or w.shape[0] % cout_mult:
        raise ValueError(f'{what} packing needs a 3x3 weight with cin % {cin_mult} == 0 and cout % {cout_mult} == 0 (and has no up2x form)')


def _packed(name, n, w, *args, dtype=torch.float32):
    packed = torch.empty(n, dtype=dtype, device=w.device)
    L.check(getattr(L.load(), name)(L.ptr(w), *args, L.ptr(packed, dtype=None), L.stream_ptr()), name)
    return packed


_WINO = {WINOGRAD: ('winograd', 'cf_pack_conv_weight_winograd', 16, None, False, True),
         WSPLIT: ('winograd f16x2', 'cf_pack_conv_weight_winograd_f16x2', 16, _f23_max, OPERAND_F16X2, True),
         WF16: ('winograd f16x2', 'cf_pack_conv_weight_winograd_f16x2', 16, _f23_max, 2, True),
         WBF16: ('winograd f16x2', 'cf_pack_conv_weight_winograd_bf16', 16, _f23_max, 1, True),
         WF43F: ('winograd F(4,3)', 'cf_pack_conv_weight_winograd43', 36, None, False, 2),
         WF43: ('winograd F(4,3) f16x2', 'cf_pack_conv_weight_winograd43_f16x2', 36, _f43_max, OPERAND_F16X2, 2)}


def _pack_winograd(w, b, code, up2x, stride2):
    what, fn, npos, domain_max, operand, wino = _WINO[code]
    _require_3x3(w, 16, 64, what, up2x)
    cout, cin = w.shape[:2]
    scale = () if domain_max is None else (pack_scale(domain_max(w)),)
    return PackedWeight(_packed(fn, npos * cin * cout, w, cout, cin, cout, cin, *scale), b, cout, cin, 9, cout, cin, bf16=operand, wino=wino, scale=(*scale, 1.0)[0])


def _pack_split(w, b, code, up2x, stride2):
    cout, cin, conv1 = w.shape[0], w.shape[1], w.dim() == 2 or tuple(w.shape[2:]) == (1, 1)
    if conv1 and (up2x or cin % 32 or cout % 64):
        raise ValueError('f16x2 1x1 packing needs cin % 32 == 0 and cout % 64 == 0')
    if not conv1:
        _require_3x3(w, 16 if stride2 else 32, 64, 'f16x2', False)
    form = 3 if conv1 else 2 if stride2 else int(bool(up2x))
    scale = pack_scale(float(w.abs().max()) * (4.0 if up2x else 1.0))
    packed = _packed('cf_pack_conv_weight_f16x2', (9, 16, 16, 1)[form] * cin * cout, w, cout, cin, form, cout, cin, scale)
    return PackedWeight(packed, b, cout, cin, 1 if conv1 else 9, cout, cin, bf16=OPERAND_F16X2, up2x=bool(up2x), scale=scale, s2=bool(stride2) and not conv1, conv1=conv1)


def _pack_gemm_split(w, b, code, up2x, stride2):
    cout, cin = w.shape[:2]
    w2 = w.reshape(cout, cin)
    if w.dim() not in (2, 4) or w.numel() != cout * cin or cout % 64 or cin % 128:
        raise ValueError('f16x2 GEMM packing needs a Linear / 1x1 weight with cout % 64 == 0 and cin % 128 == 0')
    scale = pack_scale(float(w2.abs().max()))
    return PackedWeight(_packed('cf_pack_linear_weight_f16x2', cout * cin, w2, cout, cin, scale), b, cout, cin, 1, cout, cin, bf16=OPERAND_F16X2, scale=scale)


def _pack_plain(w, b, code, up2x, stride2):
    if w.dim() not in (2, 4):
        raise ValueError('weight must be 2-D or 4-D')
    if w.dim() == 4 and (w.shape[2] != w.shape[3] or w.shape[2] not in (1, 3)):
        raise ValueError(f'unsupported kernel size {tuple(w.shape[2:])}')
    cout, cin, taps = w.shape[0], w.shape[1], 1 if w.dim() == 2 else w.shape[2] * w.shape[3]
    cout_pad, cin_pad = _cout_pad(cout), (cin + 15) // 16 * 16
    packed = _packed('cf_pack_conv_weight', L.load().cf_packed_weight_elems(cin_pad, taps, cout_pad), w, cout, cin, taps, cout_pad, cin_pad)
    return PackedWeight(packed, b, cout, cin, taps, cout_pad, cin_pad)


def _pack_16_or_folded(w, b, code, up2x, stride2):
    cout, cin, slab = w.shape[0], w.shape[1], 32 if code else 16
    if w.dim() != 4 or tuple(w.shape[2:]) != (3, 3) or cin % slab:
        raise ValueError(f"{('fp32', 'bf16', 'f16')[code]}{' up2x' if up2x else ''} packing needs a 3x3 weight with cin % {slab} == 0")
    cout_pad = _cout_pad(cout) if (code == 2 and not up2x) else max(64, _cout_pad(cout))
    name = 'cf_pack_conv_weight' + ('_up2x' if up2x else '') + ('', '_bf16', '_f16')[code]
    packed = _packed(name, (16 if up2x else 9) * cin * cout_pad, w, cout, cin, *(() if up2x else (9,)), cout_pad, cin, dtype=(torch.float32, torch.bfloat16, torch.float16)[code])
    return PackedWeight(packed, b, cout, cin, 9, cout_pad, cin, bf16=code, up2x=bool(up2x))


def pack_weight(weight, bias=None, bf16=False, up2x=False, f16=False, stride2=False):
    code = 2 if f16 else int(bf16)
    w = _f32(weight.detach()).contiguous()
    b = None if bias is None else _f32(bias.detach()).contiguous().clone()
    if stride2 and (code != SPLIT or up2x) and code != GSPLIT and code not in _WINO:
        raise ValueError('stride2 packing exists for the split-half kernel (bf16=SPLIT) only')
    packer = _pack_gemm_split if code == GSPLIT else _pack_winograd if code in _WINO else _pack_split if code == SPLIT else \
        _pack_16_or_folded if (code or up2x) else _pack_plain
    return packer(w, b, code, up2x, stride2)


def pack_weight_cat(weights, biases):
    w = torch.cat([x.detach().reshape(x.shape[0], x.shape[1]) for x in weights], dim=0)
    b = None if biases is None else torch.cat([x.detach() for x in biases], dim=0)
    return pack_weight(w, b)


def _nhwc_ld(t, what):
    B, H, W, C = t.shape
    ld = t.stride(2) if W > 1 else (t.stride(1) if H > 1 else max(C, t.stride(0) // max(H * W, 1)))
    ok = t.stride(3) == 1 and ld >= C and (W == 1 or t.stride(2) == ld) and (H == 1 or t.stride(1) == W * ld) and \
        (B == 1 or t.stride(0) == H * W * ld)
    if not ok:
        raise ValueError(f'{what}: expected a dense NHWC tensor or a channel slice of one, got shape {tuple(t.shape)} '
                         f'strides {t.stride()}')
    return ld


SPLITK_MAX = 8
SPLITK_IN_WORKGROUP = -1
GEMM_IN_WG_MAX_OUTPUTS = 1 << 20
_COUNTERS = {}


def splitk_for(pw, ho, wo, cin, batch=1):
    if (pw.bf16 and not pw.wino and pw.taps != 1) or ho * wo > 1024 or cin % 128:
        return 0
    if pw.wino == 2:
        return 0
    if pw.wino:
        if ho % 8 or wo % 16 or ho * wo > 256:
            return 0
        tiles = batch * (ho // 8) * (wo // 16) * (pw.cout_pad // 64)
    elif pw.taps == 1 and (ho * wo) % 64 == 0 and pw.cout_pad % 64 == 0:
        if int(pw.bf16) == OPERAND_F16X2 and not pw.conv1 and batch * ho * wo * pw.cout_pad <= GEMM_IN_WG_MAX_OUTPUTS and cin <= 1024:
            return SPLITK_IN_WORKGROUP
        tiles = batch * (ho * wo // 64) * (pw.cout_pad // 64)
    else:
        return 0
    cap = 256 if pw.wino else 128
    v = cin // 128
    for ns in (8, 4, 2):
        if ns <= SPLITK_MAX and v % ns == 0 and tiles * ns <= cap:
            return ns
    return 1


def _counters(device, n):
    key = (str(device), torch.cuda.current_stream(device).cuda_stream)
    t = _COUNTERS.get(key)
    if t is None or t.numel() < n:
        t = torch.zeros(max(n, 4096), dtype=torch.int32, device=device)
        _COUNTERS[key] = t
    return t


def _roofline_kind(pw, io, stride, upsample, c0, in_nchw, out_nchw, out_pixels, split_k):
    kind = ('conv3x3_s2' if stride == 2 else ('conv_up2x' if upsample else ('conv3x3_wino' if pw.wino else 'conv3x3'))) if pw.taps == 9 else 'gemm1x1'
    if pw.taps == 9 and stride == 1 and ((in_nchw and c0 <= 4) or (out_nchw and pw.cout <= 4)):
        kind = 'conv3x3_io'
    if pw.bf16:
        kind += ('', '_bf16', '_f16', '_f16x2')[int(pw.bf16)]
    if io == torch.bfloat16 and not pw.bf16:
        kind += '_bf16io'
    if pw.conv1:
        kind = 'conv1x1_stream_f16x2'
    if pw.wino == 2:
        return 'conv3x3_wino43_f16x2' if pw.bf16 else 'conv3x3_wino43'
    return kind + ('_8w' if pw.wino and pw.bf16 and pw.cout % 128 == 0 and out_pixels >= 1024 and not split_k else '')


def conv2d(x, pw, *, x2=None, stride=1, upsample=False, prologue=PRO_NONE, scale=None, shift=None,
           epilogue=EPI_NONE, res=None, sft_scale=None, sft_w=0.0, in_nchw=False, out_nchw=False, emit_stats=False,
           out=None, pad_mode=PAD_ZERO, pad_lo=0, split_k=None, act=None, x_alt=None, alt_from=0, stats_into=None,
           img_in=None, img_out=None):
    lib = L.load()
    u8_in = u8_out = None
    if img_in is not None and img_out is not None:
        raise ValueError('conv2d: img_in and img_out belong to two different layers (the first and the last conv)')
    for t, what in ((img_in, 'img_in'), (img_out, 'img_out')):
        if t is not None and (t.dim() != 4 or t.shape[3] != 3):
            raise ValueError(f'{what}: expected a uint8 (B,H,W,3) BGR image, got shape {tuple(t.shape)}')
    if img_in is not None:
        if x is not None or not in_nchw:
            raise ValueError('img_in stands for the NCHW input: pass x=None and in_nchw=True')
        u8_in = L.ptr(img_in, dtype=torch.uint8)
        B, H, W, c0 = img_in.shape
        io, ld0, dev = torch.float32, 0, img_in.device
    elif in_nchw:
        io, dev = _act_dtype(x, 'x'), x.device
        _f32(x)
        B, c0, H, W = x.shape
        ld0 = 0
        if not x.is_contiguous():
            raise ValueError('in_nchw input must be contiguous')
    else:
        io, dev = _act_dtype(x, 'x'), x.device
        B, H, W, c0 = x.shape
        ld0 = _nhwc_ld(x, 'x')
    c1 = ld1 = 0
    if x2 is not None:
        if img_in is not None or x2.shape[:3] != x.shape[:3]:
            raise ValueError('x2 spatial shape mismatch')
        c1 = x2.shape[3]
        if x2.dtype != io:
            raise TypeError(f'x2 is {x2.dtype}, x is {io}: both halves of a concatenated input share the storage type (ops.to_bf16)')
        ld1 = _nhwc_ld(x2, 'x2')
    if c0 + c1 != pw.cin and not (c1 == 0 and c0 == pw.cin_pad):
        raise ValueError(f'input channels {c0}+{c1} != weight cin {pw.cin}')
    f43_up = bool(upsample) and pw.wino == 2 and not pw.bf16
    if bool(upsample) != bool(pw.up2x) and not f43_up:
        raise ValueError('conv2d(upsample=True) needs a weight packed with up2x=True, or the fp32 F(4,3) packing (and vice versa)')
    if pw.taps == 1 and int(pw.bf16) == OPERAND_F16X2 and bool(pw.conv1) != (H * W > TOKEN_IMAGE_MAX):
        raise ValueError(f'1x1 with f16x2 operands: images of more than {TOKEN_IMAGE_MAX} pixels take a weight packed with bf16=SPLIT, '
                         'token matrices one packed with bf16=GSPLIT')
    if bool(pw.s2) != (stride == 2 and int(pw.bf16) == OPERAND_F16X2):
        raise ValueError('a weight packed with stride2=True serves conv2d(stride=2) only (and f16x2 operands at stride 2 need it)')
    if stride == 2:
        Ho, Wo = H // 2, W // 2
    else:
        Ho, Wo = (H * 2, W * 2) if upsample else (H, W)
    shape = (B, pw.cout, Ho, Wo) if out_nchw else (B, Ho, Wo, pw.cout)
    ldo = 0
    odt = torch.float32 if out_nchw else io
    if img_out is not None:
        if not out_nchw or out is not None or tuple(img_out.shape) != (B, Ho, Wo, pw.cout) or img_out.device != dev:
            raise ValueError(f'img_out stands for the NCHW output: pass out_nchw=True, no out, and a uint8 {(B, Ho, Wo, 3)} image on {dev}')
        u8_out = L.ptr(img_out, dtype=torch.uint8)
        out = img_out
    elif out is None:
        out = torch.empty(shape, dtype=odt, device=dev)
    else:
        if tuple(out.shape) != shape or out.dtype != odt or out.device != dev:
            raise ValueError(f'out: expected {odt} {shape} on {dev}')
        if out_nchw:
            if not out.is_contiguous():
                raise ValueError('out_nchw destination must be contiguous')
        else:
            ldo = _nhwc_ld(out, 'out')
    for t in (res, sft_scale):
        if t is not None and tuple(t.shape) != (B, Ho, Wo, pw.cout):
            raise ValueError(f'epilogue operand shape {tuple(t.shape)} != {(B, Ho, Wo, pw.cout)}')
        if t is not None and t.dtype != io:
            raise TypeError(f'epilogue operand is {t.dtype}, the launch stores {io}')
        if t is not None and _nhwc_ld(t, 'epilogue operand') != (ldo or pw.cout):
            raise ValueError('epilogue operands must have the channel stride of the output')
    for t in (scale, shift):
        if t is not None and tuple(t.shape) != (B, c0 + c1):
            raise ValueError(f'prologue table shape {tuple(t.shape)} != {(B, c0 + c1)}')
    d = L.ConvDesc(
        in0=None if img_in is not None else L.ptr(x, not in_nchw, dtype=io), in1=L.ptr(x2, True, dtype=io), c0=c0, c1=c1, batch=B, hin=H, win=W, hout=Ho, wout=Wo, cout=pw.cout,
        cout_pad=pw.cout_pad, taps=pw.taps, stride=stride, upsample=int(bool(upsample)), in_nchw=int(bool(in_nchw)),
        out_nchw=int(bool(out_nchw)), prologue=prologue, epilogue=epilogue, pro_scale=L.ptr(scale),
        pro_shift=L.ptr(shift), weight=L.ptr(pw.w, dtype=None), bias=L.ptr(pw.bias), res=L.ptr(res, True, dtype=io),
        sft_scale=L.ptr(sft_scale, True, dtype=io), sft_w=float(sft_w), out=None if img_out is not None else L.ptr(out, not out_nchw, dtype=odt), bf16_mfma=int(pw.bf16),
        ld_in0=ld0, ld_in1=ld1, ld_out=ldo, pad_mode=int(pad_mode), pad_lo=int(pad_lo), winograd=int(pw.wino),
        acc_scale=1.0 / pw.scale, io_bf16=int(io == torch.bfloat16))
    if x_alt is not None:
        if tuple(x_alt.shape) != tuple(x.shape) or x_alt.dtype != torch.float32 or int(pw.bf16) != OPERAND_F16X2 or pw.taps != 1 or pw.conv1 or x2 is not None:
            raise ValueError('x_alt: a second float32 token matrix of the same shape, for a split-half token GEMM (bf16=GSPLIT weight)')
        d.in0_alt, d.alt_cout0 = L.ptr(x_alt), int(alt_from)
    if act is not None and needs_act_scale(pw):
        if tuple(act.shape) != (B, 2) or prologue not in (PRO_NONE, PRO_LEAKY):
            raise ValueError('act: expected a (B, 2) table and a none / leaky prologue')
        d.act_scale = L.ptr(act)
    if split_k is None:
        dense = not in_nchw and not out_nchw and ld0 == c0 and (c1 == 0 or ld1 == c1) and ldo in (0, pw.cout)
        split_k = splitk_for(pw, Ho, Wo, c0 + c1, B) if (stride == 1 and dense) else 0
    if split_k:
        d.split_k = int(split_k)
        if split_k > 1:
            nbytes, tiles = lib.cf_conv2d_workspace_bytes(ctypes.byref(d)), lib.cf_conv2d_tiles(ctypes.byref(d))
            if nbytes < 0 or tiles <= 0:
                raise RuntimeError(f'cf_conv2d_workspace_bytes failed: {L.last_error()}')
            ws = torch.empty(nbytes // 4, dtype=torch.float32, device=dev)
            d.workspace, d.counters = L.ptr(ws), L.ptr(_counters(dev, tiles), dtype=torch.int32)
    if emit_stats and not out_nchw and pw.cout % GN_GROUPS == 0 and pw.cout // GN_GROUPS >= 2:
        d.stats_cpg = pw.cout // GN_GROUPS
        parts = lib.cf_conv2d_stats_parts(ctypes.byref(d))
        if parts <= 0:
            raise RuntimeError(f'cf_conv2d_stats_parts failed ({parts}): {L.last_error()}')
        n_part = B * GN_GROUPS * parts * 2
        part = torch.empty(n_part, dtype=torch.float64, device=dev) if stats_into is None else stats_into.take(n_part, dev)
        d.stats_out = L.ptr(part, dtype=torch.float64)
        out._cf_stats = GNStats(part, parts, d.stats_cpg)

    def launch():
        if u8_in is None and u8_out is None:
            L.check(lib.cf_conv2d(ctypes.byref(d), L.stream_ptr()), 'cf_conv2d')
        else:
            L.check(lib.cf_conv2d_u8(ctypes.byref(d), u8_in, u8_out, L.stream_ptr()), 'cf_conv2d_u8')
    if PROFILE is None:
        launch()
        return out
    e0, e1 = torch.cuda.Event(enable_timing=True), torch.cuda.Event(enable_timing=True)
    e0.record()
    launch()
    e1.record()
    x = img_in if img_in is not None else x
    cin = c0 + c1
    flops = 2.0 * B * Ho * Wo * pw.cout * cin * (4 if (upsample and not pw.wino) else pw.taps)
    esz = x.element_size()
    nbytes = float(esz * (x.numel() + (0 if x2 is None else x2.numel()) + (0 if res is None else res.numel()) + (0 if sft_scale is None else sft_scale.numel()))
                   + 4 * pw.cout * cin * pw.taps + out.element_size() * out.numel())
    kind = _roofline_kind(pw, io, stride, upsample, c0, in_nchw, out_nchw, Ho * Wo, split_k)
    PROFILE.append((kind, flops, nbytes, e0, e1, (B, H, W, cin, pw.cout)))
    return out


def linear(x, pw, *, epilogue=EPI_NONE, res=None, x_alt=None, alt_from=0):
    M, K = x.shape
    if M % 256:
        raise ValueError(f'linear: rows {M} must be a multiple of 256')
    r4 = None if res is None else res.view(M // 256, 16, 16, pw.cout)
    y = conv2d(x.view(M // 256, 16, 16, K), pw, epilogue=epilogue, res=r4, x_alt=None if x_alt is None else x_alt.view(M // 256, 16, 16, K), alt_from=alt_from)
    return y.view(M, pw.cout)


FINALIZE_FUSED = os.environ.get('CODEFORMER_HIP_FINALIZE_FUSED', '1') != '0'


def groupnorm_tables(xs, gamma, beta, eps=GN_EPS, groups=GN_GROUPS, act_growth=None):
    lib = L.load()
    B, H, W, _ = xs[0].shape
    ctot = sum(t.shape[3] for t in xs)
    if ctot % groups:
        raise ValueError(f'{ctot} channels not divisible by {groups} groups')
    cpg = ctot // groups
    hw = H * W
    dev = xs[0].device
    scale = torch.empty(B, ctot, dtype=torch.float32, device=dev)
    shift = torch.empty_like(scale)
    g_ptr, b_ptr, sc_ptr, sh_ptr = L.ptr(gamma), L.ptr(beta), L.ptr(scale), L.ptr(shift)
    stats = []
    for t in xs:
        _act_dtype(t)
        c = t.shape[3]
        if c % cpg:
            raise ValueError('concat boundary splits a group')
        st = getattr(t, '_cf_stats', None)
        if st is None or cpg % st.cpg:
            nblk = max(1, min(256, (hw * c * 4 + (1 << 17) - 1) >> 17))
            part = torch.empty(B * (c // cpg) * nblk * 2, dtype=torch.float64, device=dev)
            _f32(t)
            L.check(lib.cf_groupnorm_stats(L.ptr(t), B, hw, c, cpg, L.ptr(part, dtype=torch.float64), nblk, L.stream_ptr()), 'cf_groupnorm_stats')
            st = GNStats(part, nblk, cpg)
            stats.append((st, False))
        else:
            stats.append((st, True))
    if FINALIZE_FUSED and len(xs) <= 2:
        want_act = act_growth is not None and RANGE_SCALE and all(own for _, own in stats)
        act = torch.empty(B, 2, dtype=torch.float32, device=dev) if want_act else None
        cells = L.ptr(_act_cells(dev, B), dtype=torch.int32) if want_act else None
        sa, ca = stats[0][0], xs[0].shape[3]
        sb, cb = (stats[1][0], xs[1].shape[3]) if len(xs) == 2 else (None, 0)
        L.check(lib.cf_groupnorm_finalize2(L.ptr(sa.part, dtype=torch.float64), sa.parts, ca, sa.cpg, cpg // sa.cpg,
                                           None if sb is None else L.ptr(sb.part, dtype=torch.float64), 0 if sb is None else sb.parts, cb,
                                           1 if sb is None else sb.cpg, 1 if sb is None else cpg // sb.cpg, B, hw * cpg, g_ptr, b_ptr, float(eps),
                                           sc_ptr, sh_ptr, ctot, float(act_growth or 0.0), cells, L.ptr(act), L.stream_ptr()), 'cf_groupnorm_finalize2')
        if want_act:
            _park_act(xs, float(act_growth), act)
        return scale, shift
    coff = 0
    for t, (st, _) in zip(xs, stats):
        c = t.shape[3]
        L.check(lib.cf_groupnorm_finalize(L.ptr(st.part, dtype=torch.float64), B, st.parts, c, st.cpg, cpg // st.cpg, hw * cpg,
                                          g_ptr + 4 * coff, b_ptr + 4 * coff, float(eps), sc_ptr + 4 * coff,
                                          sh_ptr + 4 * coff, ctot, L.stream_ptr()), 'cf_groupnorm_finalize')
        coff += c
    return scale, shift


def _act_key(x, growth):
    ver = tensor_version(x)
    if ver is None and getattr(x, '_cf_stats', None) is not None:
        ver = 'inference'
    return None if ver is None else (float(growth), ver)


def _park_act(xs, growth, act):
    k0 = _act_key(xs[0], growth)
    if k0 is None:
        return
    if len(xs) == 1:
        xs[0]._cf_act = (k0, act)
    else:
        k1 = _act_key(xs[1], growth)
        if k1 is not None:
            xs[0]._cf_act_pair = (k0, k1, weakref.ref(xs[1]), act)


def layernorm(x, gamma, beta, eps=1e-5, pos=None):
    lib = L.load()
    rows, C = x.shape
    y = torch.empty_like(x)
    ypos = torch.empty_like(x) if pos is not None else None
    npos = 0 if pos is None else pos.shape[0]
    L.check(lib.cf_layernorm(L.ptr(_f32(x)), rows, C, L.ptr(gamma), L.ptr(beta), float(eps), L.ptr(pos), npos, L.ptr(y),
                             L.ptr(ypos), L.stream_ptr()), 'cf_layernorm')
    return (y, ypos) if pos is not None else y


def attention(q, k, v, batch, heads, head_dim, scale):
    lib = L.load()
    rows = batch * 256
    for t in (q, k, v):
        if t.shape[0] != rows or t.stride(1) != 1 or t.shape[1] != heads * head_dim:
            raise ValueError('attention operand must be (batch*256, heads*head_dim) with unit column stride')
    out = torch.empty(rows, heads * head_dim, dtype=torch.float32, device=q.device)
    L.check(lib.cf_attention(q.data_ptr(), q.stride(0), k.data_ptr(), k.stride(0), v.data_ptr(), v.stride(0),
                             L.ptr(out), out.stride(0), batch, heads, head_dim, 256, float(scale), L.stream_ptr()),
            'cf_attention')
    return out


def argmax_rows(logits):
    lib = L.load()
    rows, n = logits.shape
    idx = torch.empty(rows, dtype=torch.int64, device=logits.device)
    L.check(lib.cf_argmax_rows(L.ptr(_f32(logits)), rows, n, L.ptr(idx, dtype=torch.int64), L.stream_ptr()), 'cf_argmax_rows')
    return idx


def argmax_rows_gap(logits, rows_per_group):
    lib = L.load()
    rows, n = logits.shape
    rows_per_group = int(rows_per_group)
    if rows_per_group <= 0 or rows % rows_per_group:
        raise ValueError(f'argmax_rows_gap: {rows} rows are not a multiple of rows_per_group={rows_per_group}')
    idx = torch.empty(rows, dtype=torch.int64, device=logits.device)
    gap = torch.empty(rows, dtype=torch.float32, device=logits.device)
    gmin = torch.empty(rows // rows_per_group, dtype=torch.float32, device=logits.device)
    L.check(lib.cf_argmax_rows_gap(L.ptr(_f32(logits)), rows, n, rows_per_group, L.ptr(idx, dtype=torch.int64), L.ptr(gap), L.ptr(gmin),
                                   L.stream_ptr()), 'cf_argmax_rows_gap')
    return idx, gap, gmin


def codebook_gather(idx, codebook, batch, ntok, lq=None, eps=1e-5):
    lib = L.load()
    ncodes, dim = codebook.shape
    out = torch.empty(batch, ntok, dim, dtype=torch.float32, device=codebook.device)
    L.check(lib.cf_codebook_gather_adain(L.ptr(idx, dtype=torch.int64), L.ptr(_f32(codebook)), ncodes, L.ptr(lq), batch, ntok, dim,
                                         int(lq is not None), float(eps), L.ptr(out), L.stream_ptr()),
            'cf_codebook_gather_adain')
    return out


def vq_nearest(z_tokens, codebook, pw_codebook=None):
    lib = L.load()
    rows, dim = z_tokens.shape
    ncodes = codebook.shape[0]
    pw = pw_codebook or pack_weight(codebook)
    scores = linear(z_tokens, pw)
    zz = torch.empty(rows, dtype=torch.float32, device=z_tokens.device)
    ee = torch.empty(ncodes, dtype=torch.float32, device=z_tokens.device)
    L.check(lib.cf_row_sqnorm(L.ptr(z_tokens), rows, dim, L.ptr(zz), L.stream_ptr()), 'cf_row_sqnorm')
    L.check(lib.cf_row_sqnorm(L.ptr(_f32(codebook)), ncodes, dim, L.ptr(ee), L.stream_ptr()), 'cf_row_sqnorm')
    idx = torch.empty(rows, dtype=torch.int64, device=z_tokens.device)
    dmin = torch.empty(rows, dtype=torch.float32, device=z_tokens.device)
    L.check(lib.cf_vq_argmin(L.ptr(scores), L.ptr(zz), L.ptr(ee), rows, ncodes, L.ptr(idx, dtype=torch.int64), L.ptr(dmin), L.stream_ptr()),
            'cf_vq_argmin')
    return idx, dmin, (scores, zz, ee)


def to_nhwc(x):
    lib = L.load()
    B, C, H, W = x.shape
    x = _f32(x).contiguous()
    y = torch.empty(B, H, W, C, dtype=torch.float32, device=x.device)
    L.check(lib.cf_nchw_to_nhwc(L.ptr(x), B, C, H * W, L.ptr(y), L.stream_ptr()), 'cf_nchw_to_nhwc')
    return y


def pixel_unshuffle_nhwc(x, scale, c_pad=None):
    lib = L.load()
    B, C, Hs, Ws = x.shape
    if Hs % scale or Ws % scale:
        raise ValueError(f'pixel_unshuffle: {Hs}x{Ws} not divisible by {scale}')
    cu = C * scale * scale
    c_pad = (cu + 15) // 16 * 16 if c_pad is None else c_pad
    x = _f32(x).contiguous()
    y = torch.empty(B, Hs // scale, Ws // scale, c_pad, dtype=torch.float32, device=x.device)
    L.check(lib.cf_pixel_unshuffle_nhwc(L.ptr(x), B, C, Hs // scale, Ws // scale, scale, c_pad, L.ptr(y), L.stream_ptr()),
            'cf_pixel_unshuffle_nhwc')
    return y


def to_nchw(x):
    lib = L.load()
    B, H, W, C = x.shape
    y = torch.empty(B, C, H, W, dtype=torch.float32, device=x.device)
    L.check(lib.cf_nhwc_to_nchw(L.ptr(_f32(x)), B, C, H * W, L.ptr(y), L.stream_ptr()), 'cf_nhwc_to_nchw')
    return y


def img_u8_to_tensor(img):
    lib = L.load()
    B, H, W, _ = img.shape
    out = torch.empty(B, 3, H, W, dtype=torch.float32, device=img.device)
    L.check(lib.cf_img_u8_to_tensor(L.ptr(img, dtype=torch.uint8), B, H, W, L.ptr(out), L.stream_ptr()), 'cf_img_u8_to_tensor')
    return out


def tensor_to_img_u8(t):
    lib = L.load()
    B, _, H, W = t.shape
    img = torch.empty(B, H, W, 3, dtype=torch.uint8, device=t.device)
    L.check(lib.cf_tensor_to_img_u8(L.ptr(_f32(t).contiguous()), B, H, W, L.ptr(img, dtype=torch.uint8), L.stream_ptr()), 'cf_tensor_to_img_u8')
    return img


def mask_composite(x, y):
    lib = L.load()
    B, _, H, W = x.shape
    out = torch.empty_like(x)
    L.check(lib.cf_mask_composite(L.ptr(_f32(x).contiguous()), L.ptr(_f32(y).contiguous()), B, H, W, L.ptr(out), L.stream_ptr()),
            'cf_mask_composite')
    return out


_FBA_DTYPES = {torch.float32: 0, torch.float16: 1, torch.bfloat16: 2}


def fused_bias_act(x, bias, negative_slope=0.2, scale=math.sqrt(2.0), ref=None, act=3, grad=0):
    lib = L.load()
    if x.dtype not in _FBA_DTYPES:
        raise TypeError(f'fused_bias_act: float32 / float16 / bfloat16 tensors (got {x.dtype})')
    x = x.contiguous()
    bias = None if bias is None or bias.numel() == 0 else bias.detach().to(x.dtype).contiguous()
    ref = None if ref is None or ref.numel() == 0 else ref.detach().to(x.dtype).contiguous()
    if ref is not None and ref.shape != x.shape:
        raise ValueError('fused_bias_act: ref must have the shape of x')
    if bias is not None and bias.numel() != x.shape[1]:
        raise ValueError('fused_bias_act: bias must have one value per channel (dim 1)')
    hw = 1
    for s in x.shape[2:]:
        hw *= s
    y = torch.empty_like(x)
    L.check(lib.cf_fused_bias_act_ex(x.data_ptr(), 0 if bias is None else bias.data_ptr(), 0 if ref is None else ref.data_ptr(),
                                     x.numel(), x.shape[1] if x.dim() > 1 else 1, hw, int(act), int(grad), float(negative_slope),
                                     float(scale), _FBA_DTYPES[x.dtype], y.data_ptr(), L.stream_ptr()), 'cf_fused_bias_act_ex')
    return y


def upfirdn2d(x, kernel, up=1, down=1, pad=(0, 0)):
    lib = L.load()
    x = _f32(x).contiguous()
    n, c, h, w = x.shape
    kh, kw = kernel.shape
    p0, p1 = pad
    oh = (h * up + p0 + p1 - kh) // down + 1
    ow = (w * up + p0 + p1 - kw) // down + 1
    y = torch.empty(n, c, oh, ow, dtype=torch.float32, device=x.device)
    L.check(lib.cf_upfirdn2d(L.ptr(x), n * c, h, w, L.ptr(_f32(kernel).contiguous()), kh, kw, up, up, down, down, p0, p1,
                             p0, p1, L.ptr(y), L.stream_ptr()), 'cf_upfirdn2d')
    return y


def _c6(m):
    vals = [float(v) for v in (m.reshape(-1).tolist() if hasattr(m, 'reshape') else m)]
    if len(vals) != 6:
        raise ValueError('affine matrix must have 6 elements')
    return (ctypes.c_double * 6)(*vals)


def warp_affine_u8(src, inv_dev, dst, region=None, border=(0, 0, 0)):
    lib = L.load()
    n, dh, dw, _ = dst.shape
    shared = src.dim() == 3
    sh, sw = (src.shape[0], src.shape[1]) if shared else (src.shape[1], src.shape[2])
    if (not shared and src.shape[0] != n) or tuple(inv_dev.shape) != (n, 6):
        raise ValueError('warp_affine_u8: batch mismatch')
    rx, ry, rw, rh = region or (0, 0, dw, dh)
    L.check(lib.cf_warp_affine_u8(L.ptr(src, dtype=torch.uint8), 0 if shared else sh * sw * 3, sh, sw, L.ptr(inv_dev, dtype=torch.float64), n,
                                  L.ptr(dst, dtype=torch.uint8), dh, dw, rx, ry, rw, rh, int(border[0]), int(border[1]), int(border[2]),
                                  L.stream_ptr()), 'cf_warp_affine_u8')
    return dst


def warp_affine_f32(src, inv, region):
    lib = L.load()
    rx, ry, rw, rh = region
    out = torch.empty(rh, rw, dtype=torch.float32, device=src.device)
    L.check(lib.cf_warp_affine_f32(L.ptr(src), src.shape[0], src.shape[1], _c6(inv), L.ptr(out), rx, ry, rw, rh, L.stream_ptr()),
            'cf_warp_affine_f32')
    return out


def erode(x, k):
    lib = L.load()
    tmp, out = torch.empty_like(x), torch.empty_like(x)
    L.check(lib.cf_erode_f32(L.ptr(x), L.ptr(tmp), L.ptr(out), x.shape[0], x.shape[1], int(k), L.stream_ptr()), 'cf_erode_f32')
    return out


def gaussian_blur(x, taps_dev, region_xy=(0, 0), frame_hw=None):
    lib = L.load()
    ch, cw = frame_hw or (x.shape[0], x.shape[1])
    tmp, out = torch.empty_like(x), torch.empty_like(x)
    L.check(lib.cf_gaussian_blur_f32(L.ptr(x), L.ptr(tmp), L.ptr(out), x.shape[0], x.shape[1], int(region_xy[0]), int(region_xy[1]), ch, cw,
                                     L.ptr(taps_dev), taps_dev.numel(), L.stream_ptr()), 'cf_gaussian_blur_f32')
    return out


def sum_partials(x, out64):
    lib = L.load()
    L.check(lib.cf_sum_f32(L.ptr(x), x.numel(), L.ptr(out64, dtype=torch.float64), L.stream_ptr()), 'cf_sum_f32')


def paste_blend(canvas, face, inv, ero, soft, region, parse=None):
    lib = L.load()
    rx, ry, rw, rh = region
    L.check(lib.cf_paste_blend(L.ptr(canvas), canvas.shape[0], canvas.shape[1], L.ptr(face, dtype=torch.uint8), face.shape[0], face.shape[1],
                               _c6(inv), L.ptr(ero), L.ptr(soft), L.ptr(parse), rx, ry, rw, rh, L.stream_ptr()), 'cf_paste_blend')


def resize_linear_u8(src, dh, dw):
    lib = L.load()
    out = torch.empty(dh, dw, 3, dtype=torch.float32, device=src.device)
    L.check(lib.cf_resize_linear_u8(L.ptr(src, dtype=torch.uint8), src.shape[0], src.shape[1], L.ptr(out), dh, dw, L.stream_ptr()),
            'cf_resize_linear_u8')
    return out


def resize_area_u8(src, dh, dw):
    lib = L.load()
    if src.dim() != 3 or src.shape[2] != 3 or not src.is_contiguous():
        raise ValueError('resize_area_u8 expects a contiguous uint8 (H, W, 3) image')
    out = torch.empty(dh, dw, 3, dtype=torch.uint8, device=src.device)
    L.check(lib.cf_resize_area_u8(L.ptr(src, dtype=torch.uint8), src.shape[0], src.shape[1], L.ptr(out, dtype=torch.uint8), dh, dw, L.stream_ptr()),
            'cf_resize_area_u8')
    return out


def f32_to_u8_trunc(x):
    lib = L.load()
    out = torch.empty(x.shape, dtype=torch.uint8, device=x.device)
    L.check(lib.cf_f32_to_u8_trunc(L.ptr(x), x.numel(), L.ptr(out, dtype=torch.uint8), L.stream_ptr()), 'cf_f32_to_u8_trunc')
    return out


def box_overlay_u8(canvas, faces_dev, face_hw):
    lib = L.load()
    out = torch.empty(canvas.shape, dtype=torch.uint8, device=canvas.device)
    n = 0 if faces_dev is None else faces_dev.shape[0]
    if n and tuple(faces_dev.shape) != (n, 11):
        raise ValueError('box_overlay_u8: faces_dev must be (n, 11)')
    L.check(lib.cf_box_overlay_u8(L.ptr(canvas), canvas.shape[0], canvas.shape[1], L.ptr(faces_dev, dtype=torch.float64) if n else None, n,
                                  int(face_hw[0]), int(face_hw[1]), L.ptr(out, dtype=torch.uint8), L.stream_ptr()), 'cf_box_overlay_u8')
    return out


def resize_linear_f32(x, dh, dw):
    lib = L.load()
    if x.dim() != 3:
        raise ValueError('resize_linear_f32 expects (n, H, W) planes')
    out = torch.empty(x.shape[0], dh, dw, dtype=torch.float32, device=x.device)
    if x.shape[0]:
        L.check(lib.cf_resize_linear_f32(L.ptr(x), x.shape[0], x.shape[1], x.shape[2], L.ptr(out), dh, dw, L.stream_ptr()),
                'cf_resize_linear_f32')
    return out


def esrgan_tile_gather(faces, pre_pad, mod, window):
    lib = L.load()
    n, h, w, _ = faces.shape
    py0, px0, th, tw = window
    out = torch.empty(n, 3, th, tw, dtype=torch.float32, device=faces.device)
    L.check(lib.cf_esrgan_tile_gather_u8(L.ptr(faces, dtype=torch.uint8), n, h, w, int(pre_pad), int(mod), py0, px0, th, tw, L.ptr(out),
                                         L.stream_ptr()), 'cf_esrgan_tile_gather_u8')
    return out


def esrgan_tile_scatter(up, core, out, dst_yx):
    lib = L.load()
    n, _, uh, uw = up.shape
    oy, ox, ch, cw = core
    if out.shape[0] != n:
        raise ValueError('esrgan_tile_scatter: batch mismatch')
    L.check(lib.cf_esrgan_tile_scatter_u8(L.ptr(up), n, uh, uw, oy, ox, ch, cw, L.ptr(out, dtype=torch.uint8), out.shape[1], out.shape[2],
                                          int(dst_yx[0]), int(dst_yx[1]), L.stream_ptr()), 'cf_esrgan_tile_scatter_u8')


def label_lut(labels, lut):
    lib = L.load()
    out = torch.empty(labels.shape, dtype=torch.float32, device=labels.device)
    arr = (ctypes.c_float * len(lut))(*[float(v) for v in lut])
    L.check(lib.cf_label_lut_f32(L.ptr(labels, dtype=torch.int64), labels.numel(), arr, len(lut), L.ptr(out), L.stream_ptr()), 'cf_label_lut_f32')
    return out


def scale_clear_border_(x, border, scale):
    lib = L.load()
    B, H, W = x.shape
    L.check(lib.cf_scale_clear_border_f32(L.ptr(x), B, H, W, int(border), float(scale), L.stream_ptr()), 'cf_scale_clear_border_f32')
    return x
```

### include/codeformer_hip.h

```cpp
#ifndef CODEFORMER_HIP_H
#define CODEFORMER_HIP_H

#include <stdint.h>

#ifdef __cplusplus
extern "C" {
#endif

#define CF_ABI_VERSION 22
#define CF_SPLITK_IN_WORKGROUP (-1)

typedef void* cf_stream_t;

enum cf_status {
  CF_OK = 0,
  CF_ERR_ARG = -1,
  CF_ERR_LAUNCH = -2,
};

int cf_version(void);
const char* cf_build_id(void);
const char* cf_last_error(void);
int cf_device_cu_count(void);
int cf_device_init(void);

enum cf_prologue {
  CF_PRO_NONE = 0,
  CF_PRO_AFFINE = 1,
  CF_PRO_AFFINE_SWISH = 2,
  CF_PRO_LEAKY = 3,
};
enum cf_epilogue {
  CF_EPI_NONE = 0,
  CF_EPI_RESIDUAL = 1,
  CF_EPI_SFT = 2,
  CF_EPI_GELU = 3,
  CF_EPI_LEAKY = 4,
  CF_EPI_AXPY = 5,
  CF_EPI_AXPY2 = 6,
};

enum cf_operand {
  CF_OPERAND_F32 = 0,
  CF_OPERAND_BF16 = 1,
  CF_OPERAND_F16 = 2,
  CF_OPERAND_F16X2 = 3,
};

enum cf_pad {
  CF_PAD_ZERO = 0,
  CF_PAD_REFLECT = 1,
  CF_PAD_EDGE = 2,
};

typedef struct cf_conv_desc {
  const float* in0;
  const float* in1;
  int32_t c0, c1;
  int32_t batch, hin, win;
  int32_t hout, wout;
  int32_t cout;
  int32_t cout_pad;
  int32_t taps;
  int32_t stride;
  int32_t upsample;
  int32_t in_nchw;
  int32_t out_nchw;
  int32_t prologue;
  int32_t epilogue;
  const float* pro_scale;
  const float* pro_shift;
  const float* weight;
  const float* bias;
  const float* res;
  const float* sft_scale;
  float sft_w;
  float* out;
  double* stats_out;
  int32_t stats_cpg;
  int32_t bf16_mfma;
  int32_t ld_in0, ld_in1, ld_out;
  int32_t pad_mode;
  int32_t pad_lo;
  int32_t winograd;
  float acc_scale;
  int32_t split_k;
  float* workspace;
  uint32_t* counters;
  const float* act_scale;
  int32_t io_bf16;
  const float* in0_alt;
  int32_t alt_cout0;
} cf_conv_desc;

int cf_conv2d(const cf_conv_desc* d, cf_stream_t stream);
int cf_conv2d_u8(const cf_conv_desc* d, const uint8_t* img_in, uint8_t* img_out, cf_stream_t stream);
int cf_conv2d_stats_parts(const cf_conv_desc* d);
int64_t cf_conv2d_workspace_bytes(const cf_conv_desc* d);
int cf_conv2d_tiles(const cf_conv_desc* d);

int cf_pack_conv_weight(const float* w, int cout, int cin, int taps, int cout_pad, int cin_pad,
                        float* packed, cf_stream_t stream);
int64_t cf_packed_weight_elems(int cin_pad, int taps, int cout_pad);
int cf_pack_conv_weight_winograd(const float* w, int cout, int cin, int cout_pad, int cin_pad, float* packed, cf_stream_t stream);
int cf_pack_conv_weight_winograd_f16x2(const float* w, int cout, int cin, int cout_pad, int cin_pad, float scale, void* packed,
                                       cf_stream_t stream);
int cf_pack_conv_weight_winograd43_f16x2(const float* w, int cout, int cin, int cout_pad, int cin_pad, float scale, void* packed,
                                         cf_stream_t stream);
int cf_pack_conv_weight_winograd43(const float* w, int cout, int cin, int cout_pad, int cin_pad, void* packed, cf_stream_t stream);
int cf_pack_conv_weight_winograd_bf16(const float* w, int cout, int cin, int cout_pad, int cin_pad, float scale, void* packed,
                                      cf_stream_t stream);
int cf_pack_linear_weight_f16x2(const float* w, int n, int k, float scale, void* packed, cf_stream_t stream);
int cf_pack_conv_weight_bf16(const float* w, int cout, int cin, int taps, int cout_pad, int cin_pad, void* packed,
                             cf_stream_t stream);
int cf_pack_conv_weight_up2x(const float* w, int cout, int cin, int cout_pad, int cin_pad, float* packed, cf_stream_t stream);
int cf_pack_conv_weight_up2x_bf16(const float* w, int cout, int cin, int cout_pad, int cin_pad, void* packed,
                                  cf_stream_t stream);
int cf_pack_conv_weight_f16(const float* w, int cout, int cin, int taps, int cout_pad, int cin_pad, void* packed,
                            cf_stream_t stream);
int cf_pack_conv_weight_up2x_f16(const float* w, int cout, int cin, int cout_pad, int cin_pad, void* packed,
                                 cf_stream_t stream);
int cf_pack_conv_weight_f16x2(const float* w, int cout, int cin, int up2x, int cout_pad, int cin_pad, float scale, void* packed,
                              cf_stream_t stream);

int cf_groupnorm_stats(const float* x, int batch, int hw, int c, int cpg, double* partial, int parts,
                       cf_stream_t stream);
int cf_act_scale_from_stats(const double* partial, int batch, int nper, float growth, float* scratch, float* act, cf_stream_t stream);
int cf_act_scale_from_tensor(const float* x, int batch, int64_t n_per_image, float growth, float* scratch, float* act, cf_stream_t stream);
int cf_act_scale_fused(const double* partial_a, int nper_a, const double* partial_b, int nper_b, const float* x, int64_t n_per_image, int batch,
                       float growth, uint32_t* cells, float* act, cf_stream_t stream);
int cf_groupnorm_finalize(const double* partial, int batch, int parts, int c, int cpg, int gmerge, int64_t count,
                          const float* gamma, const float* beta, float eps, float* scale, float* shift, int ld,
                          cf_stream_t stream);
int cf_groupnorm_finalize2(const double* partial_a, int parts_a, int c_a, int cpg_a, int gmerge_a, const double* partial_b, int parts_b, int c_b,
                           int cpg_b, int gmerge_b, int batch, int64_t count, const float* gamma, const float* beta, float eps, float* scale,
                           float* shift, int ld, float act_growth, uint32_t* cells, float* act, cf_stream_t stream);

int cf_layernorm(const float* x, int rows, int c, const float* gamma, const float* beta, float eps,
                 const float* pos, int npos, float* y, float* ypos, cf_stream_t stream);

int cf_attention(const float* q, int ldq, const float* k, int ldk, const float* v, int ldv, float* out, int ldo,
                 int batch, int heads, int head_dim, int nkeys, float scale, cf_stream_t stream);

int cf_argmax_rows(const float* logits, int rows, int n, int64_t* idx, cf_stream_t stream);
int cf_argmax_rows_gap(const float* logits, int rows, int n, int rows_per_group, int64_t* idx, float* gap, float* group_min_gap,
                       cf_stream_t stream);

int cf_codebook_gather_adain(const int64_t* idx, const float* codebook, int codebook_size, const float* lq,
                             int batch, int ntok, int dim, int adain, float eps, float* out, cf_stream_t stream);

int cf_row_sqnorm(const float* x, int rows, int dim, float* out, cf_stream_t stream);
int cf_vq_argmin(const float* scores, const float* zz, const float* ee, int rows, int ncodes, int64_t* idx,
                 float* dist_min, cf_stream_t stream);

int cf_nchw_to_nhwc(const float* x, int batch, int c, int hw, float* y, cf_stream_t stream);
int cf_nhwc_to_nchw(const float* x, int batch, int c, int hw, float* y, cf_stream_t stream);

int cf_pixel_unshuffle_nhwc(const float* x, int batch, int c, int h, int w, int s, int c_pad, float* out, cf_stream_t stream);

int cf_img_u8_to_tensor(const uint8_t* img, int batch, int h, int w, float* out, cf_stream_t stream);
int cf_tensor_to_img_u8(const float* t, int batch, int h, int w, uint8_t* img, cf_stream_t stream);
int cf_mask_composite(const float* x, const float* y, int batch, int h, int w, float* out, cf_stream_t stream);
int cf_f32_to_bf16(const float* x, int64_t numel, void* out, cf_stream_t stream);

int cf_fused_bias_act(const float* x, const float* bias, int64_t numel, int c, int hw, float slope, float scale,
                      float* y, cf_stream_t stream);
int cf_fused_bias_act_ex(const void* x, const void* bias, const void* ref, int64_t numel, int c, int hw, int act, int grad, float alpha,
                         float scale, int dtype, void* y, cf_stream_t stream);
int cf_upfirdn2d(const float* x, int nplanes, int in_h, int in_w, const float* kernel, int kh, int kw, int up_x,
                 int up_y, int down_x, int down_y, int pad_x0, int pad_x1, int pad_y0, int pad_y1, float* y,
                 cf_stream_t stream);

int cf_warp_affine_u8(const uint8_t* src, int64_t src_stride, int sh, int sw, const double* inv_dev, int n, uint8_t* dst, int dh, int dw,
                      int rx, int ry, int rw, int rh, int b0, int b1, int b2, cf_stream_t stream);
int cf_warp_affine_f32(const float* src, int sh, int sw, const double* inv_host, float* dst_region, int rx, int ry, int rw, int rh,
                       cf_stream_t stream);
int cf_erode_f32(const float* in_region, float* tmp_region, float* out_region, int rh, int rw, int k, cf_stream_t stream);
int cf_gaussian_blur_f32(const float* in_region, float* tmp_region, float* out_region, int rh, int rw, int rx, int ry, int ch, int cw,
                         const float* taps_dev, int ksize, cf_stream_t stream);
int cf_sum_f32(const float* x, int64_t n, double* partials64, cf_stream_t stream);
int cf_paste_blend(float* canvas, int ch, int cw, const uint8_t* face, int fh, int fw, const double* inv_host, const float* ero_region,
                   const float* soft_region, const float* parse_region, int rx, int ry, int rw, int rh, cf_stream_t stream);
int cf_resize_linear_u8(const uint8_t* src, int sh, int sw, float* dst, int dh, int dw, cf_stream_t stream);
int cf_resize_area_u8(const uint8_t* src, int sh, int sw, uint8_t* dst, int dh, int dw, cf_stream_t stream);
int cf_f32_to_u8_trunc(const float* src, int64_t n, uint8_t* dst, cf_stream_t stream);
int cf_label_lut_f32(const int64_t* labels, int64_t n, const float* lut_host, int nlut, float* out, cf_stream_t stream);
int cf_scale_clear_border_f32(float* x, int batch, int h, int w, int border, float scale, cf_stream_t stream);
int cf_box_overlay_u8(const float* canvas, int ch, int cw, const double* faces_dev, int nfaces, int fh, int fw, uint8_t* out,
                      cf_stream_t stream);
int cf_resize_linear_f32(const float* src, int batch, int sh, int sw, float* dst, int dh, int dw, cf_stream_t stream);
int cf_esrgan_tile_gather_u8(const uint8_t* faces, int n, int h, int w, int pre_pad, int mod, int py0, int px0, int th, int tw, float* out,
                             cf_stream_t stream);
int cf_esrgan_tile_scatter_u8(const float* up, int n, int uh, int uw, int oy, int ox, int ch, int cw, uint8_t* out, int oh, int ow, int dy,
                              int dx, cf_stream_t stream);

#ifdef __cplusplus
}
#endif
#endif
```

Before: 342.3 faces/s.

## Use sub-pixel Winograd F(4,2) for fp32 upsample convolutions

Replaces the upsample+3x3 conv path, which ran Winograd F(4,3) over a gathered 2x-nearest input, with a sub-pixel decomposition. Each of the four output phases folds the 3x3 kernel into a 2x2 kernel, applied with Winograd F(4,2) on the low-resolution input. This needs 25 transform positions per phase instead of 36 and avoids gathering the duplicated upsampled pixels. It adds a new weight packing (100 positions), new input/output transforms, phase-strided output stores, and a tighter shape constraint (multiples of 32). The different transform constants may also shift fp32 rounding.

```diff
diff --git a/codeformer_amd/archs/vqgan_arch.py b/codeformer_amd/archs/vqgan_arch.py
--- a/codeformer_amd/archs/vqgan_arch.py
+++ b/codeformer_amd/archs/vqgan_arch.py
@@ -111,7 +111,7 @@
             bf16 = ops.SPLIT
         c = self.conv.in_channels
         if int(bf16) == ops.WINOGRAD_F43 and x.dtype == torch.float32 and ops.f43_up_ok(c, self.conv.out_channels, 2 * x.shape[1], 2 * x.shape[2]):
-            pw = self._packed(('conv', 'f43up'), lambda: ops.pack_weight(self.conv.weight, self.conv.bias, bf16=ops.WF43F), self.conv.weight, self.conv.bias)
+            pw = self._packed(('conv', 'f42up'), lambda: ops.pack_weight(self.conv.weight, self.conv.bias, bf16=ops.WF42U), self.conv.weight, self.conv.bias)
             return ops.conv2d(x, pw, upsample=True, emit_stats=True)
         pw = self._pw_conv('conv', bf16, up2x=True, hw=x.shape[1:3])
         return ops.conv2d(x, pw, upsample=True, emit_stats=True, act=ops.act_scale(x) if ops.needs_act_scale(pw) else None)
diff --git a/codeformer_amd/csrc/cf_wf43.hip b/codeformer_amd/csrc/cf_wf43.hip
--- a/codeformer_amd/csrc/cf_wf43.hip
+++ b/codeformer_amd/csrc/cf_wf43.hip
@@ -75,9 +75,14 @@
 
 __device__ __forceinline__ unsigned f4_vu(unsigned lq, unsigned p, unsigned t) { return (lq & 1u) + 2u * (((t >> 1) + 4u * (lq >> 1) + p) & 7u); }
 
-template <int PRO, int EPI, int NW, int KS, bool F32, bool UP = false>
+template <int PRO, int EPI, int NW, int KS, bool F32, int UPF = 0>
 __global__ __launch_bounds__(NW * 64, 4) void wf43_kernel(const F4Args a) {
-  static_assert(!UP || (F32 && PRO == CF_PRO_NONE && EPI == CF_EPI_NONE), "the upsampling gather: fp32 operands, no prologue, no epilogue operand");
+  constexpr bool UP = UPF == 2;
+  constexpr bool GUP = UPF == 1;
+  static_assert(UPF == 0 || (F32 && NW == 16 && KS == 32 && PRO == CF_PRO_NONE && EPI == CF_EPI_NONE), "the upsampling forms: fp32 operands on 32-channel slabs, no prologue, no epilogue operand");
+  constexpr int NPW = UP ? 13 : 18;
+  constexpr int NXI = UP ? 5 : 6;
+  constexpr int OS = UP ? 2 : 1;
   static_assert(KS == 16 || (KS == 32 && NW == 16), "32-channel slabs need the LDS of the 16-wave form");
   constexpr int F4_THREADS = NW * 64;
   constexpr int F4_BN = NW * 8;
@@ -105,9 +110,13 @@
   const int n0 = ntile * F4_BN;
   const int b = mt / a.tiles_per_img;
   const int rt = mt - b * a.tiles_per_img;
-  const int tyw = rt / a.tiles_x;
+  const int blocks = a.tiles_per_img >> 2;
+  const int phase = UP ? rt / blocks : 0;
+  const int pa = phase >> 1, pb = phase & 1;
+  const int blk = UP ? rt - phase * blocks : rt;
+  const int tyw = blk / a.tiles_x;
   const int y0 = tyw * F4_TH;
-  const int x0 = (rt - tyw * a.tiles_x) * F4_TW;
+  const int x0 = (blk - tyw * a.tiles_x) * F4_TW;
   const int n = a.cin / KS;
 
   constexpr bool affine = PRO == CF_PRO_AFFINE || PRO == CF_PRO_AFFINE_SWISH;
@@ -120,14 +129,15 @@
   float act_s, act_is, act_s02;
   cf_act_scales<!affine>(a.act_scale, b, act_s, act_is, act_s02);
 
-  const int pix_origin = (y0 - 1) * a.w + (x0 - 1);
+  const int py0 = y0 - 1 + pa, px0 = x0 - 1 + pb;
+  const int pix_origin = py0 * a.w + px0;
   auto item = [&](unsigned u, int j, unsigned& rel, bool& valid) __attribute__((always_inline)) {
     const unsigned p = u + (unsigned)(PSTEP * j);
     const unsigned hy = (p * 3641u) >> 16;
     const unsigned hx = p - 18u * hy;
-    const int iy = y0 - 1 + (int)hy, ix = x0 - 1 + (int)hx;
+    const int iy = py0 + (int)hy, ix = px0 + (int)hx;
     valid = (int)(p < (unsigned)F4_NPIX) & (int)((unsigned)iy < (unsigned)a.h) & (int)((unsigned)ix < (unsigned)a.w);
-    if constexpr (UP) {
+    if constexpr (GUP) {
       const unsigned sy = valid ? (unsigned)iy : (unsigned)(y0 + 8), sx = valid ? (unsigned)ix : (unsigned)(x0 + 8);
       rel = (sy >> 1) * ((unsigned)a.w >> 1) + (sx >> 1);
     } else {
@@ -136,8 +146,8 @@
   };
   const size_t img0 = (size_t)b * a.h * a.w;
   const unsigned img_px = (unsigned)(a.h * a.w);
-  const size_t img0_in = UP ? img0 / 4 : img0;
-  const unsigned img_px_in = UP ? img_px / 4 : img_px;
+  const size_t img0_in = GUP ? img0 / 4 : img0;
+  const unsigned img_px_in = GUP ? img_px / 4 : img_px;
   const __amdgpu_buffer_rsrc_t rs_in0 = f4_rsrc(a.in0 + img0_in * a.c0, img_px_in * (unsigned)a.c0 * 4u);
   const __amdgpu_buffer_rsrc_t rs_in1 = f4_rsrc(a.c1 ? a.in1 + img0_in * a.c1 : a.in0, img_px_in * (unsigned)a.c1 * 4u);
   constexpr bool HALVES = F4_APT >= 6;
@@ -157,7 +167,7 @@
       unsigned rel;
       bool valid;
       item(tl / (unsigned)QPP, j, rel, valid);
-      const unsigned voff = (__umul24(UP ? rel : (unsigned)(pix_origin + (int)rel), cs) + k4x) * 4u;
+      const unsigned voff = (__umul24(GUP ? rel : (unsigned)(pix_origin + (int)rel), cs) + k4x) * 4u;
       (HALVES && j >= RAN ? rb[j % RAN] : ra[j % RAN]) = first ? f4_ld128(rs_in0, voff, soff) : f4_ld128(rs_in1, voff, soff);
     }
   };
@@ -213,10 +223,32 @@
       }
     }
   };
+  auto bt42 = [](auto xi, f4_f32x2 d0, f4_f32x2 d1, f4_f32x2 d2, f4_f32x2 d3, f4_f32x2 d4) __attribute__((always_inline)) {
+    constexpr int XI = decltype(xi)::value;
+    if constexpr (XI == 0) return (d0 + d3) - (d1 + d2) * 1.5f;
+    else if constexpr (XI == 1) return (d1 + d3) - d2 * 2.5f;
+    else if constexpr (XI == 2) return (d3 - d2) - d1 * 2.f;
+    else if constexpr (XI == 3) return (d2 - d1) * 0.5f + d3;
+    else return (d1 + d4) - (d2 + d3) * 1.5f;
+  };
+  auto row_pass42 = [&](const f4_f32x2 (&zz)[5], int pos) __attribute__((always_inline)) {
+    f4_f32x2 v[5];
+    v[0] = bt42(std::integral_constant<int, 0>{}, zz[0], zz[1], zz[2], zz[3], zz[4]);
+    v[1] = bt42(std::integral_constant<int, 1>{}, zz[0], zz[1], zz[2], zz[3], zz[4]);
+    v[2] = bt42(std::integral_constant<int, 2>{}, zz[0], zz[1], zz[2], zz[3], zz[4]);
+    v[3] = bt42(std::integral_constant<int, 3>{}, zz[0], zz[1], zz[2], zz[3], zz[4]);
+    v[4] = bt42(std::integral_constant<int, 4>{}, zz[0], zz[1], zz[2], zz[3], zz[4]);
+#pragma unroll
+    for (int nu = 0; nu < 5; ++nu) {
+      t_hi[(pos + nu) * PSK] = v[nu][0];
+      t_lo[(pos + nu) * PSK] = v[nu][1];
+    }
+  };
   auto transform = [&](int chunk, auto mid) __attribute__((always_inline)) {
     const char* const pb = reinterpret_cast<const char*>(smem + (chunk & 1) * PATCHF);
     unsigned ln = (unsigned)lane;
     asm volatile("" : "+v"(ln));
+    constexpr int TG0 = UP ? 15 : 18;
     const unsigned t_tile = KS == 32 ? 4u * (unsigned)(wave & 3) + (ln >> 4) : 8u * (unsigned)(wave & 1) + (ln >> 3);
     const unsigned t_cp = KS == 32 ? ln & 15u : ln & 7u;
     const unsigned t_ty = t_tile >> 2, t_tx = t_tile & 3u;
@@ -229,25 +261,50 @@
     if (F32) {
       const unsigned lq0 = (2u * t_cp) & 3u, j = t_cp >> 1;
       if (KS == 32) {
-        t_hi = V + (tg * 18) * PSK + t_tile * 32 + f4_vu(lq0, j >> 1, t_tile) * 2u + (j & 1u);
-        t_lo = V + (tg * 18) * PSK + t_tile * 32 + f4_vu(lq0 + 1u, j >> 1, t_tile) * 2u + (j & 1u);
+        t_hi = V + (tg * TG0) * PSK + t_tile * 32 + f4_vu(lq0, j >> 1, t_tile) * 2u + (j & 1u);
+        t_lo = V + (tg * TG0) * PSK + t_tile * 32 + f4_vu(lq0 + 1u, j >> 1, t_tile) * 2u + (j & 1u);
       } else {
-        t_hi = V + (tg * 18) * PSK + t_tile * CF_BK + ((lq0 ^ (unsigned)f4_vs((int)t_ty)) << 2) + j;
-        t_lo = V + (tg * 18) * PSK + t_tile * CF_BK + (((lq0 + 1u) ^ (unsigned)f4_vs((int)t_ty)) << 2) + j;
+        t_hi = V + (tg * TG0) * PSK + t_tile * CF_BK + ((lq0 ^ (unsigned)f4_vs((int)t_ty)) << 2) + j;
+        t_lo = V + (tg * TG0) * PSK + t_tile * CF_BK + (((lq0 + 1u) ^ (unsigned)f4_vs((int)t_ty)) << 2) + j;
       }
     } else if (KS == 32) {
       const unsigned lq = t_cp >> 2, e = t_cp & 3u;
-      t_hi = V + (tg * 18) * PSK + t_tile * 32 + f4_vu(lq, e >> 1, t_tile) * 2u + (e & 1u);
-      t_lo = V + (tg * 18) * PSK + t_tile * 32 + f4_vu(lq, 2u + (e >> 1), t_tile) * 2u + (e & 1u);
+      t_hi = V + (tg * TG0) * PSK + t_tile * 32 + f4_vu(lq, e >> 1, t_tile) * 2u + (e & 1u);
+      t_lo = V + (tg * TG0) * PSK + t_tile * 32 + f4_vu(lq, 2u + (e >> 1), t_tile) * 2u + (e & 1u);
     } else {
-      t_hi = V + (tg * 18) * PSK + t_tile * CF_BK + (((t_cp >> 1) ^ (unsigned)f4_vs((int)t_ty)) << 2) + (t_cp & 1u);
+      t_hi = V + (tg * TG0) * PSK + t_tile * CF_BK + (((t_cp >> 1) ^ (unsigned)f4_vs((int)t_ty)) << 2) + (t_cp & 1u);
       t_lo = t_hi + 2;
     }
     auto px = [&](int r, int j) __attribute__((always_inline)) {
       const int q = 2 * r + j;
       return *reinterpret_cast<const f4_f32x2*>(pb + (4 << SH) * (4 * r + (q >> 2)) + (tk[q >> 2] ^ (((unsigned)q & 3u) << SH)));
     };
-    if (tg == 0) {
+    if constexpr (UP) {
+      auto xi_pass = [&](auto xi) __attribute__((always_inline)) {
+        constexpr int XI = decltype(xi)::value;
+        f4_f32x2 z[5];
+#pragma unroll
+        for (int j = 0; j < 5; ++j) {
+          const f4_f32x2 zero = {0.f, 0.f};
+          z[j] = bt42(xi, XI == 0 ? px(0, j) : zero, px(1, j), px(2, j), px(3, j), XI == 4 ? px(4, j) : zero);
+        }
+        __builtin_amdgcn_sched_barrier(0);
+        row_pass42(z, (XI >= 3 ? XI - 3 : XI) * 5);
+        __builtin_amdgcn_sched_barrier(0);
+      };
+      if (tg == 0) {
+        xi_pass(std::integral_constant<int, 0>{});
+        xi_pass(std::integral_constant<int, 1>{});
+        mid();
+        __builtin_amdgcn_sched_barrier(0);
+        xi_pass(std::integral_constant<int, 2>{});
+      } else {
+        xi_pass(std::integral_constant<int, 3>{});
+        mid();
+        __builtin_amdgcn_sched_barrier(0);
+        xi_pass(std::integral_constant<int, 4>{});
+      }
+    } else if (tg == 0) {
       {
         f4_f32x2 z[6];
 #pragma unroll
@@ -303,10 +360,10 @@
   };
 
   const int m_g = wave / (NW / 2), m_nb = wave % (NW / 2);
-  f32x4 acc[18];
-#pragma unroll
-  for (int i = 0; i < 18; ++i) acc[i] = f32x4{0.f, 0.f, 0.f, 0.f};
-  const __amdgpu_buffer_rsrc_t rs_w = f4_rsrc(a.weight, 36u * (unsigned)a.cin * (unsigned)a.cout * 4u);
+  f32x4 acc[NPW];
+#pragma unroll
+  for (int i = 0; i < NPW; ++i) acc[i] = f32x4{0.f, 0.f, 0.f, 0.f};
+  const __amdgpu_buffer_rsrc_t rs_w = f4_rsrc(a.weight, (UP ? 100u : 36u) * (unsigned)a.cin * (unsigned)a.cout * 4u);
   const unsigned w_pos = (unsigned)a.cin * (unsigned)a.cout * 4u;
   const unsigned w_chunk = (unsigned)(a.cout * KS) * 4u;
   const unsigned w_s0 = (unsigned)(18 * m_g) * w_pos + (unsigned)(n0 / 16 + m_nb) * (unsigned)(64 * KS);
@@ -374,9 +431,10 @@
   };
   typedef _Float16 f4_f16x8 __attribute__((ext_vector_type(8)));
   f32x4 xb[3][2], xa[1][2];
-  const int p_g = 18 * m_g;
+  const int p_g = NPW * m_g;
   const int p_nb = m_nb;
-  const unsigned w_s32 = (unsigned)p_g * w_pos + (unsigned)(n0 / 16 + p_nb) * (unsigned)(64 * KS);
+  const bool p_last = !UP || m_g == 0;
+  const unsigned w_s32 = (unsigned)(p_g + 25 * phase) * w_pos + (unsigned)(n0 / 16 + p_nb) * (unsigned)(64 * KS);
   auto load_B32 = [&](int chunk, int i) __attribute__((always_inline)) {
     const unsigned so = w_s32 + (unsigned)i * w_pos + (unsigned)chunk * w_chunk;
     xb[i % 3][0] = f4_ld128(rs_w, lane16, so);
@@ -404,20 +462,22 @@
     };
     read_A(0);
 #pragma unroll
-    for (int i = 0; i < 18; ++i) {
+    for (int i = 0; i < NPW; ++i) {
       __builtin_amdgcn_sched_barrier(0);
       if (F32) {
-#pragma unroll
-        for (int j = 0; j < 8; ++j) {
-          acc[i] = __builtin_amdgcn_mfma_f32_16x16x4f32(xa[0][j >> 2][j & 3], xb[i % 3][j >> 2][j & 3], acc[i], 0, 0, 0);
+        if (i + 1 < NPW || p_last) {
+#pragma unroll
+          for (int j = 0; j < 8; ++j) {
+            acc[i] = __builtin_amdgcn_mfma_f32_16x16x4f32(xa[0][j >> 2][j & 3], xb[i % 3][j >> 2][j & 3], acc[i], 0, 0, 0);
+          }
         }
       } else {
         mf(xa[0][1], xb[i % 3][0], acc[i]);
         mf(xa[0][0], xb[i % 3][1], acc[i]);
         mf(xa[0][0], xb[i % 3][0], acc[i]);
       }
-      if (i + 1 < 18) read_A(i + 1);
-      if (i + 3 < 18) load_B32(chunk, i + 3);
+      if (i + 1 < NPW && (p_last || i + 1 < NPW - 1)) read_A(i + 1);
+      if (i + 3 < NPW && (p_last || i + 3 < NPW - 1)) load_B32(chunk, i + 3);
       __builtin_amdgcn_sched_barrier(0);
     }
   };
@@ -554,10 +614,10 @@
   const int nn = n0 + 2 * e_cp;
   f4_f32x2 bias2 = {0.f, 0.f};
   if (a.bias) bias2 = *reinterpret_cast<const f4_f32x2*>(a.bias + nn);
-  const unsigned e_rowc = (unsigned)a.w * (unsigned)a.cout * 4u;
-  const unsigned e_px = (unsigned)a.cout * 4u;
-  const unsigned e_img = img_px * (unsigned)a.cout * 4u;
-  const __amdgpu_buffer_rsrc_t rs_out = f4_rsrc(a.out + img0 * a.cout, e_img);
+  const unsigned e_rowc = (unsigned)(OS * OS * a.w) * (unsigned)a.cout * 4u;
+  const unsigned e_px = (unsigned)(OS * a.cout) * 4u;
+  const unsigned e_img = (unsigned)(OS * OS) * img_px * (unsigned)a.cout * 4u;
+  const __amdgpu_buffer_rsrc_t rs_out = f4_rsrc(a.out + (size_t)(OS * OS) * img0 * a.cout, e_img);
   const __amdgpu_buffer_rsrc_t rs_res = f4_rsrc(EPI == CF_EPI_NONE ? a.out : a.res + img0 * a.cout, e_img);
   const __amdgpu_buffer_rsrc_t rs_sft = f4_rsrc(EPI == CF_EPI_SFT ? a.sft_scale + img0 * a.cout : a.out, e_img);
   const bool rh1 = e_rh != 0;
@@ -568,7 +628,8 @@
     unsigned e_zero = 0;
     asm volatile("" : "+v"(e_zero));
     const unsigned voff0 = (unsigned)(2 * e_rh) * e_rowc + (unsigned)(2 * e_cp) * 4u + e_zero;
-    const unsigned soff0 = (unsigned)(y0 + 4 * (e_tp >> 1)) * e_rowc + (unsigned)(x0 + 4 * (2 * th + (e_tp & 1))) * e_px + (unsigned)n0 * 4u;
+    const unsigned soff0 = (unsigned)(y0 + 4 * (e_tp >> 1)) * e_rowc + (unsigned)(x0 + 4 * (2 * th + (e_tp & 1))) * e_px + (unsigned)n0 * 4u +
+                           (UP ? (unsigned)(pa * 2 * a.w + pb) * (unsigned)a.cout * 4u : 0u);
     f4_f32x2 r0[2][4], r1[2][4];
 #pragma unroll
     for (int aa = 0; aa < 2; ++aa)
@@ -580,8 +641,8 @@
     __builtin_amdgcn_sched_barrier(0);
     if (th > 0) __syncthreads();
 #pragma unroll
-    for (int i = 0; i < 18; ++i) {
-      float* mp = Mst + ((18 * m_g + i) * 8 + 2 * (lane >> 4)) * F4_BN + m_nb * 16 + (lane & 15);
+    for (int i = 0; i < NPW; ++i) {
+      float* mp = Mst + ((NPW * m_g + i) * 8 + 2 * (lane >> 4)) * F4_BN + m_nb * 16 + (lane & 15);
       mp[0] = acc[i][2 * th];
       mp[F4_BN] = acc[i][2 * th + 1];
     }
@@ -594,7 +655,16 @@
     __syncthreads();
     const float* mq = Mst + e_tp * F4_BN + 2 * e_cp;
     auto col = [&](int nu, f4_f32x2& tA, f4_f32x2& tB) __attribute__((always_inline)) {
-      auto m = [&](int xi) __attribute__((always_inline)) { return *reinterpret_cast<const f4_f32x2*>(mq + ((xi * 6 + nu) * 8) * F4_BN); };
+      auto m = [&](int xi) __attribute__((always_inline)) { return *reinterpret_cast<const f4_f32x2*>(mq + ((xi * NXI + nu) * 8) * F4_BN); };
+      if constexpr (UP) {
+        const f4_f32x2 m1 = m(1), m2 = m(2), m3 = m(3);
+        const f4_f32x2 me = *reinterpret_cast<const f4_f32x2*>(mq + (((rh1 ? 4 : 0) * NXI + nu) * 8) * F4_BN);
+        const f4_f32x2 x = m1 + m2 * ca1 + m3 * ca2, y = (m2 * cb1 + m3 * cb2) - m1;
+        const f4_f32x2 xm = x + me, ym = y + me;
+        tA = rh1 ? x : xm;
+        tB = rh1 ? ym : y;
+        return;
+      }
       const f4_f32x2 m1 = m(1), m2 = m(2), m3 = m(3), m4 = m(4);
       const f4_f32x2 me = *reinterpret_cast<const f4_f32x2*>(mq + (((rh1 ? 5 : 0) * 6 + nu) * 8) * F4_BN);
       const f4_f32x2 s1 = m1 + m2, d1 = m1 - m2, s2 = m3 + m4, d2 = m3 - m4;
@@ -604,7 +674,18 @@
       tB = rh1 ? ym : y;
     };
     f4_f32x2 o[2][4];
-    {
+    if constexpr (UP) {
+      f4_f32x2 t[5][2];
+#pragma unroll
+      for (int nu = 0; nu < 5; ++nu) col(nu, t[nu][0], t[nu][1]);
+#pragma unroll
+      for (int aa = 0; aa < 2; ++aa) {
+        o[aa][0] = (t[0][aa] + t[1][aa]) + (t[2][aa] + t[3][aa]);
+        o[aa][1] = (t[2][aa] * 0.5f + t[3][aa] * 2.f) - t[1][aa];
+        o[aa][2] = (t[2][aa] * 0.25f + t[3][aa] * 4.f) + t[1][aa];
+        o[aa][3] = ((t[2][aa] * 0.125f + t[3][aa] * 8.f) - t[1][aa]) + t[4][aa];
+      }
+    } else {
       f4_f32x2 t0[2], ta[2], tb[2];
       col(0, t0[0], t0[1]);
       col(1, ta[0], ta[1]);
@@ -762,6 +843,32 @@
   packed[i] = out;
 }
 
+__global__ void pack_weight_wf42_up_kernel(const float* __restrict__ w, int cout, int cin, int nchunks, float* __restrict__ packed, long total) {
+  const long i = (long)blockIdx.x * blockDim.x + threadIdx.x;
+  if (i >= total) return;
+  const int j = (int)(i & 7), ln = (int)((i >> 3) & 63);
+  long r = i >> 9;
+  const int ntiles = cout / 16;
+  const int nn = (int)(r % ntiles) * 16 + (ln & 15);
+  r /= ntiles;
+  const int chunk = (int)(r % nchunks);
+  r /= nchunks;
+  const int pos = (int)(r % 25), phase = (int)(r / 25);
+  const int c = chunk * 32 + 4 * j + (ln >> 4);
+  const int xi = pos / 5, nu = pos % 5, pa = phase >> 1, pb = phase & 1;
+  const double G[5][2] = {{1.0, 0.0}, {-2.0 / 9.0, 2.0 / 9.0}, {-8.0 / 9.0, -4.0 / 9.0}, {1.0 / 9.0, 2.0 / 9.0}, {0.0, 1.0}};
+  const float* g = w + ((long)nn * cin + c) * 9;
+  double f[2][2] = {{0.0, 0.0}, {0.0, 0.0}};
+#pragma unroll
+  for (int y = 0; y < 3; ++y)
+#pragma unroll
+    for (int x = 0; x < 3; ++x) f[(y + 1 - pa) >> 1][(x + 1 - pb) >> 1] += (double)g[y * 3 + x];
+  double u = 0.0;
+#pragma unroll
+  for (int y = 0; y < 2; ++y) u += G[xi][y] * (f[y][0] * G[nu][0] + f[y][1] * G[nu][1]);
+  packed[i] = (float)u;
+}
+
 }
 
 static int f4_wide_mode() {
@@ -803,14 +910,29 @@
   return CF_OK;
 }
 
+extern "C" int cf_pack_conv_weight_winograd42_up(const float* w, int cout, int cin, int cout_pad, int cin_pad, void* packed, cf_stream_t stream) {
+  CF_REQUIRE(w && packed, "cf_pack_conv_weight_winograd42_up: null pointer");
+  CF_REQUIRE(cin_pad == cin && cout_pad == cout && cin > 0 && cout > 0 && cin % 32 == 0 && cout % 128 == 0,
+             "cf_pack_conv_weight_winograd42_up: bad padding cin %d->%d cout %d->%d (cin %% 32 == 0, cout %% 128 == 0, no padding)", cin, cin_pad, cout, cout_pad);
+  CF_REQUIRE(f4_k32_enabled(), "cf_pack_conv_weight_winograd42_up: the sub-pixel form runs on 32-channel slabs (CF_F43_WIDE=k16 is set)");
+  const long total = 100L * cin * cout;
+  hipLaunchKernelGGL(pack_weight_wf42_up_kernel, dim3((unsigned)((total + 255) / 256)), dim3(256), 0, (hipStream_t)stream, w, cout, cin, cin / 32,
+                     reinterpret_cast<float*>(packed), total);
+  CF_CHECK_LAUNCH("cf_pack_conv_weight_winograd42_up");
+  return CF_OK;
+}
+
 int cf_wf43_launch(const cf_conv_desc* d, hipStream_t stream, int* parts_query) {
   CF_REQUIRE(d->taps == 9 && d->stride == 1 && !d->in_nchw && !d->out_nchw &&
                  (d->bf16_mfma == CF_OPERAND_F16X2 || d->bf16_mfma == CF_OPERAND_F32),
              "cf_conv2d(winograd 2): F(4x4,3x3) covers 3x3 stride-1 NHWC convolutions with split-half or fp32 operands");
   const bool f32 = d->bf16_mfma == CF_OPERAND_F32;
+  const bool sub = d->upsample == 2;
   CF_REQUIRE(!d->upsample || (f32 && d->prologue == CF_PRO_NONE && d->epilogue == CF_EPI_NONE && d->c1 == 0 && d->cout % 128 == 0 && d->c0 % 32 == 0 &&
                               f4_k32_enabled()),
              "cf_conv2d(winograd 2, upsample): fp32 operands, one input with c0 %% 32 == 0, cout %% 128 == 0, no prologue / epilogue operand");
+  CF_REQUIRE(!sub || (d->hin % F4_TH == 0 && d->win % F4_TW == 0 && d->hout == 2 * d->hin && d->wout == 2 * d->win),
+             "cf_conv2d(winograd 2, upsample 2): needs an input of %dx%d multiples (got %dx%d)", F4_TH, F4_TW, d->hin, d->win);
   if (!f32)
     if (const int e = cf_require_acc_scale(d, "cf_conv2d(winograd 2)")) return e;
   CF_REQUIRE(!f32 || !d->act_scale, "cf_conv2d(winograd 2): fp32 operands take no activation range scale");
@@ -843,6 +965,11 @@
   CF_REQUIRE(!k32 || d->c0 % 32 == 0, "cf_conv2d(winograd 2): with cout %% 128 == 0 and cin %% 32 == 0 the concat boundary must be a multiple of 32 (c0 = %d)", d->c0);
   a.ntn = d->cout / (wide ? 128 : 64);
   a.nt_out = cf_nt_store((long)d->batch * d->hout * d->wout * d->cout * 4);
+  if (sub) {
+    a.h = d->hin;
+    a.w = d->win;
+    a.tiles_x = d->win / F4_TW;
+  }
   if (parts_query) {
     *parts_query = a.nparts;
     return CF_OK;
@@ -850,9 +977,11 @@
   const size_t lds = (k32 ? F4_LDS_FLOATS_32 : wide ? F4_LDS_FLOATS_16 : F4_LDS_FLOATS) * sizeof(float);
   const dim3 grid(a.tiles_per_img * d->batch * a.ntn), block(wide ? 1024 : 512);
   if (d->upsample) {
-    CF_LDS_ATTR((wf43_kernel<CF_PRO_NONE, CF_EPI_NONE, 16, 32, true, true>), F4_LDS_FLOATS_32 * sizeof(float));
-    hipLaunchKernelGGL((wf43_kernel<CF_PRO_NONE, CF_EPI_NONE, 16, 32, true, true>), grid, block, lds, stream, a);
-    CF_CHECK_LAUNCH("cf_conv2d(winograd F(4,3) fp32, upsampling gather)");
+    CF_LDS_ATTR((wf43_kernel<CF_PRO_NONE, CF_EPI_NONE, 16, 32, true, 1>), F4_LDS_FLOATS_32 * sizeof(float));
+    CF_LDS_ATTR((wf43_kernel<CF_PRO_NONE, CF_EPI_NONE, 16, 32, true, 2>), F4_LDS_FLOATS_32 * sizeof(float));
+    if (sub) hipLaunchKernelGGL((wf43_kernel<CF_PRO_NONE, CF_EPI_NONE, 16, 32, true, 2>), grid, block, lds, stream, a);
+    else hipLaunchKernelGGL((wf43_kernel<CF_PRO_NONE, CF_EPI_NONE, 16, 32, true, 1>), grid, block, lds, stream, a);
+    CF_CHECK_LAUNCH("cf_conv2d(winograd F(4,3) / F(4,2) fp32, upsampling forms)");
     return CF_OK;
   }
   auto launch = [&](auto pro, auto epi, auto op) {
diff --git a/codeformer_amd/lib.py b/codeformer_amd/lib.py
--- a/codeformer_amd/lib.py
+++ b/codeformer_amd/lib.py
@@ -62,6 +62,7 @@
     'cf_pack_conv_weight_winograd_bf16': (_I, [_P, _I, _I, _I, _I, _F, _P, _P]),
     'cf_pack_conv_weight_winograd43_f16x2': (_I, [_P, _I, _I, _I, _I, _F, _P, _P]),
     'cf_pack_conv_weight_winograd43': (_I, [_P, _I, _I, _I, _I, _P, _P]),
+    'cf_pack_conv_weight_winograd42_up': (_I, [_P, _I, _I, _I, _I, _P, _P]),
     'cf_pack_linear_weight_f16x2': (_I, [_P, _I, _I, _F, _P, _P]),
     'cf_pack_conv_weight_up2x_bf16': (_I, [_P, _I, _I, _I, _I, _P, _P]),
     'cf_pack_conv_weight_up2x_f16': (_I, [_P, _I, _I, _I, _I, _P, _P]),
diff --git a/codeformer_amd/ops.py b/codeformer_amd/ops.py
--- a/codeformer_amd/ops.py
+++ b/codeformer_amd/ops.py
@@ -80,6 +80,7 @@
 WF43 = 11
 WINOGRAD_F43 = 12
 WF43F = 13
+WF42U = 14
 OPERAND_F16X2 = 3
 SPLIT_CODES = (SPLIT, SPLIT_F43)
 
@@ -114,7 +115,7 @@
 
 
 def f43_up_ok(cin, cout, hout, wout):
-    return cin % 32 == 0 and cin <= 256 and cout % 128 == 0 and hout % 16 == 0 and wout % 16 == 0 and \
+    return cin % 32 == 0 and cin <= 256 and cout % 128 == 0 and hout % 32 == 0 and wout % 32 == 0 and \
         hout * wout >= F43_WIDE_MIN_PIXELS_FP32
 
 
@@ -273,6 +274,23 @@
     return float(torch.einsum('xa,kcab,yb->kcxy', Gm, w.double(), Gm).abs().max())
 
 
+B42T = ((1.0, -1.5, -1.5, 1.0, 0.0), (0.0, 1.0, -2.5, 1.0, 0.0), (0.0, -2.0, -1.0, 1.0, 0.0), (0.0, -0.5, 0.5, 1.0, 0.0), (0.0, 1.0, -1.5, -1.5, 1.0))
+G42 = ((1.0, 0.0), (-2 / 9, 2 / 9), (-8 / 9, -4 / 9), (1 / 9, 2 / 9), (0.0, 1.0))
+A42T = ((1.0, 1.0, 1.0, 1.0, 0.0), (0.0, -1.0, 0.5, 2.0, 0.0), (0.0, 1.0, 0.25, 4.0, 0.0), (0.0, -1.0, 0.125, 8.0, 1.0))
+
+
+def fold_phase_taps(w, a, b):
+    def fold(t, p, dim):
+        g0, g1, g2 = t.unbind(dim)
+        return torch.stack((g0, g1 + g2) if p == 0 else (g0 + g1, g2), dim)
+    return fold(fold(w, a, -2), b, -1)
+
+
+def f42_weights(w):
+    G = torch.tensor(G42, dtype=torch.float64, device=w.device)
+    return torch.stack([torch.einsum('xa,kcab,yb->kcxy', G, fold_phase_taps(w.double(), p >> 1, p & 1), G) for p in range(4)])
+
+
 def _require_3x3(w, cin_mult, cout_mult, what, up2x):
     if up2x or w.dim() != 4 or tuple(w.shape[2:]) != (3, 3) or w.shape[1] % cin_mult or w.shape[0] % cout_mult:
         raise ValueError(f'{what} packing needs a 3x3 weight with cin % {cin_mult} == 0 and cout % {cout_mult} == 0 (and has no up2x form)')
@@ -289,15 +307,17 @@
          WF16: ('winograd f16x2', 'cf_pack_conv_weight_winograd_f16x2', 16, _f23_max, 2, True),
          WBF16: ('winograd f16x2', 'cf_pack_conv_weight_winograd_bf16', 16, _f23_max, 1, True),
          WF43F: ('winograd F(4,3)', 'cf_pack_conv_weight_winograd43', 36, None, False, 2),
+         WF42U: ('winograd F(4,2) sub-pixel', 'cf_pack_conv_weight_winograd42_up', 100, None, False, 2),
          WF43: ('winograd F(4,3) f16x2', 'cf_pack_conv_weight_winograd43_f16x2', 36, _f43_max, OPERAND_F16X2, 2)}
 
 
 def _pack_winograd(w, b, code, up2x, stride2):
     what, fn, npos, domain_max, operand, wino = _WINO[code]
-    _require_3x3(w, 16, 64, what, up2x)
+    up = code == WF42U
+    _require_3x3(w, 32 if up else 16, 128 if up else 64, what, up2x)
     cout, cin = w.shape[:2]
     scale = () if domain_max is None else (pack_scale(domain_max(w)),)
-    return PackedWeight(_packed(fn, npos * cin * cout, w, cout, cin, cout, cin, *scale), b, cout, cin, 9, cout, cin, bf16=operand, wino=wino, scale=(*scale, 1.0)[0])
+    return PackedWeight(_packed(fn, npos * cin * cout, w, cout, cin, cout, cin, *scale), b, cout, cin, 9, cout, cin, bf16=operand, up2x=up, wino=wino, scale=(*scale, 1.0)[0])
 
 
 def _pack_split(w, b, code, up2x, stride2):
@@ -461,9 +481,10 @@
         ld1 = _nhwc_ld(x2, 'x2')
     if c0 + c1 != pw.cin and not (c1 == 0 and c0 == pw.cin_pad):
         raise ValueError(f'input channels {c0}+{c1} != weight cin {pw.cin}')
-    f43_up = bool(upsample) and pw.wino == 2 and not pw.bf16
+    f43_up = bool(upsample) and pw.wino == 2 and not pw.bf16 and not pw.up2x
+    f42_up = bool(upsample) and pw.wino == 2 and not pw.bf16 and bool(pw.up2x)
     if bool(upsample) != bool(pw.up2x) and not f43_up:
-        raise ValueError('conv2d(upsample=True) needs a weight packed with up2x=True, or the fp32 F(4,3) packing (and vice versa)')
+        raise ValueError('conv2d(upsample=True) needs a weight packed with up2x=True, or the fp32 F(4,3) / F(4,2) sub-pixel packing (and vice versa)')
     if pw.taps == 1 and int(pw.bf16) == OPERAND_F16X2 and bool(pw.conv1) != (H * W > TOKEN_IMAGE_MAX):
         raise ValueError(f'1x1 with f16x2 operands: images of more than {TOKEN_IMAGE_MAX} pixels take a weight packed with bf16=SPLIT, '
                          'token matrices one packed with bf16=GSPLIT')
@@ -503,7 +524,7 @@
             raise ValueError(f'prologue table shape {tuple(t.shape)} != {(B, c0 + c1)}')
     d = L.ConvDesc(
         in0=None if img_in is not None else L.ptr(x, not in_nchw, dtype=io), in1=L.ptr(x2, True, dtype=io), c0=c0, c1=c1, batch=B, hin=H, win=W, hout=Ho, wout=Wo, cout=pw.cout,
-        cout_pad=pw.cout_pad, taps=pw.taps, stride=stride, upsample=int(bool(upsample)), in_nchw=int(bool(in_nchw)),
+        cout_pad=pw.cout_pad, taps=pw.taps, stride=stride, upsample=2 if f42_up else int(bool(upsample)), in_nchw=int(bool(in_nchw)),
         out_nchw=int(bool(out_nchw)), prologue=prologue, epilogue=epilogue, pro_scale=L.ptr(scale),
         pro_shift=L.ptr(shift), weight=L.ptr(pw.w, dtype=None), bias=L.ptr(pw.bias), res=L.ptr(res, True, dtype=io),
         sft_scale=L.ptr(sft_scale, True, dtype=io), sft_w=float(sft_w), out=None if img_out is not None else L.ptr(out, not out_nchw, dtype=odt), bf16_mfma=int(pw.bf16),
diff --git a/include/codeformer_hip.h b/include/codeformer_hip.h
--- a/include/codeformer_hip.h
+++ b/include/codeformer_hip.h
@@ -108,6 +108,7 @@
 int cf_pack_conv_weight_winograd43_f16x2(const float* w, int cout, int cin, int cout_pad, int cin_pad, float scale, void* packed,
                                          cf_stream_t stream);
 int cf_pack_conv_weight_winograd43(const float* w, int cout, int cin, int cout_pad, int cin_pad, void* packed, cf_stream_t stream);
+int cf_pack_conv_weight_winograd42_up(const float* w, int cout, int cin, int cout_pad, int cin_pad, void* packed, cf_stream_t stream);
 int cf_pack_conv_weight_winograd_bf16(const float* w, int cout, int cin, int cout_pad, int cin_pad, float scale, void* packed,
                                       cf_stream_t stream);
 int cf_pack_linear_weight_f16x2(const float* w, int n, int k, float scale, void* packed, cf_stream_t stream);
```

Measured after the change: 350.5 faces/s, median of 6. 1.02x the previous value.
